# dannyfa/VAE-GAM

Hardware: AMD Instinct MI355X
Metric: fMRI volumes/sec/train-step (41x49x35) (higher is better)
Workload: dtype f32; 1 GPU; configs[2] full VAE-GAM: B=64/GPU C=8, 41x49x35, 2 subj x 98 vol synthetic checker, fwd+bwd+Adam, hipGraph replay; global_batch=64, covariates=8, parallelism=dp1

## Files before the change

include/vaegam.h:

```cpp
#ifndef VAEGAM_H
#define VAEGAM_H
#include <stdint.h>
#ifdef __cplusplus
extern "C" {
#endif

typedef struct vg_conv_desc {
    int32_t N;
    int32_t CI, CO;
    int32_t ID, IH, IW;
    int32_t OD, OH, OW;
    int32_t KD, KH, KW;
    int32_t stride;
    int32_t pad_d, pad_h, pad_w;
    int32_t relu_in;
    int32_t per_group;
} vg_conv_desc;

int         vg_version(void);
const char* vg_last_error(void);

int vg_corr3d(const vg_conv_desc* d, const float* x, const float* wpk, const float* bias,
              const float* in_scale, const float* in_shift, const float* mask_src, float* y, void* stream);

int vg_tconv3d_s2(const vg_conv_desc* d, const float* x, const float* wpk, const float* bias,
                  const float* in_scale, const float* in_shift, const float* mask_src, float* y, void* stream);
int64_t vg_tconv3d_s2_stats_chunks(const vg_conv_desc* d, int32_t stats_per_group);
int vg_tconv3d_s2_stats(const vg_conv_desc* d, const float* x, const float* wpk, const float* bias,
                        const float* in_scale, const float* in_shift, float* y, int32_t stats_per_group,
                        int32_t stats_relu, double* stats_part, void* stream);

typedef struct vg_mm_desc {
    int32_t N, CI, CO;
    int32_t ID, IH, IW, OD, OH, OW;
    int32_t nq, ks[4];
    int32_t PDT, PH, PW, PD;
    int32_t sdi, shi, swi, d0, LD, cc;
    int32_t sdo, sho, swo, od0[4], oh0[4], ow0[4];
    int32_t relu_in, per_group, tpc, slack;
    int32_t dbuf;
    int32_t PHB;
    int32_t hlo, hhi;
    int32_t waves;
} vg_mm_desc;
int64_t vg_conv_mm_stats_chunks(const vg_mm_desc* d, int32_t stats_per_group);
int vg_conv_mm(const vg_mm_desc* d, const float* x, const float* a_img, const int32_t* tau, const int32_t* dlt, const float* bias,
               const float* in_scale, const float* in_shift, const float* mask_src, float* y, int32_t stats_per_group,
               int32_t stats_relu, double* stats_part, void* stream);
int vg_gather_f32(const float* src, const int32_t* idx, float* dst, int64_t n, void* stream);

typedef struct vg_wgrad_desc {
    int32_t N, CB, CA;
    int32_t PD, PH, PW;
    int32_t AD, AH, AW;
    int32_t KD, KH, KW;
    int32_t stride;
    int32_t pad_d, pad_h, pad_w;
    int32_t pro_on_a;
    int32_t relu_in;
    int32_t per_group;
} vg_wgrad_desc;
int64_t vg_wgrad3d_ws_bytes(const vg_wgrad_desc* d);
int vg_wgrad3d(const vg_wgrad_desc* d, const float* a, const float* b, const float* in_scale,
               const float* in_shift, float* ws, float* dw, int32_t accumulate, void* stream);

int64_t vg_wgrad3d_grouped_ws_bytes(const vg_wgrad_desc* d);
int vg_wgrad3d_grouped(const vg_wgrad_desc* d, const float* a, const float* b, const float* in_scale,
                       const float* in_shift, float* ws, float* out, void* stream);

int64_t vg_bn_ws_bytes(int32_t N, int32_t C, int64_t P, int32_t per_group);
int vg_bn_stats(const float* x, int32_t N, int32_t C, int64_t P, int32_t per_group, int32_t relu,
                const float* gamma, const float* beta, float eps, void* ws, double* ext_sums,
                float* scale, float* shift, float* mean, float* rstd, void* stream);
int vg_bn_finalize(const double* sums, int32_t G, int32_t C, const float* gamma, const float* beta,
                   float eps, float* scale, float* shift, float* mean, float* rstd, void* stream);
int vg_bn_stats_from_parts(const double* part, int32_t G, int32_t C, int64_t chunks, double count,
                           const float* gamma, const float* beta, float eps, double* ext_sums, double* sums_ws,
                           float* scale, float* shift, float* mean, float* rstd, void* stream);

int vg_bn_bwd_reduce(const float* dxe, const float* p, int32_t N, int32_t C, int64_t P, int32_t per_group,
                     int32_t relu, const float* mean, const float* rstd, void* ws, double* sums, void* stream);
int vg_bn_bwd_apply(float* dxe_inout, const float* p, int32_t N, int32_t C, int64_t P, int32_t per_group,
                    int32_t relu, const float* gamma, const float* mean, const float* rstd,
                    const double* sums, double count, float* dgamma_part, float* dbeta_part,
                    void* ws, float* chsum, int32_t chsum_accumulate, void* stream);

int64_t vg_bn_tconv1_ws_bytes(int32_t N, int32_t C, int32_t ID, int32_t per_group);
int vg_bn_bwd_reduce_tconv1(const float* dy, const float* w, const float* p, int32_t N, int32_t C, int32_t ID, int32_t IH, int32_t IW,
                            int32_t per_group, int32_t relu, const float* mean, const float* rstd, void* ws, double* sums, void* stream);
int vg_bn_bwd_apply_tconv1(const float* dy, const float* w, const float* p, float* dp, int32_t N, int32_t C, int32_t ID, int32_t IH,
                           int32_t IW, int32_t per_group, int32_t relu, const float* gamma, const float* mean, const float* rstd,
                           const double* sums, double count, void* ws, float* chsum, int32_t chsum_accumulate, void* stream);

int vg_bn_tconv1_sums(const float* q, const float* w, const float* gamma, const float* beta, int32_t G, int32_t C, int32_t K,
                      double* sums, float* dw, int32_t accumulate, void* stream);

int vg_channel_sum(const float* x, int32_t N, int32_t C, int64_t P, void* ws, float* out, int32_t accumulate, void* stream);

int64_t vg_gam_ws_bytes(int32_t C, int32_t B, int64_t V);
int vg_gam_elbo_fwd(const float* logits, const float* gain, const float* x, const double* eps,
                    const float* glm, int32_t C, int32_t B, int64_t V, void* ws,
                    float* sum_log_prob, float* dist, float* maps_out, void* stream);
int vg_gam_elbo_bwd(const float* logits, const float* gain, const float* x, const double* eps,
                    const float* glm, const float* dist, const float* g_slp, const float* g_dist,
                    int32_t C, int32_t B, int64_t V, void* ws,
                    float* d_logits, float* d_gain, double* d_eps, float* d_total, int32_t total_accumulate, void* stream);

int vg_bn_param_grad(const double* sums, int32_t G, int32_t C, float* dgamma, float* dbeta, int32_t accumulate, void* stream);

int vg_data_bn_nshift(const float* mean, const float* rstd, int32_t n, float* nshift, void* stream);
int vg_data_bn_grads(const float* dw_hat, const float* db, const float* w, const float* gamma, const float* beta,
                     int32_t CO, int32_t CI, int32_t taps, float* dw, float* dbias, float* dgamma, float* dbeta,
                     int32_t accumulate, void* stream);

int vg_latent_fwd(const float* mu, const float* w, const float* a, const float* eps_w, const float* eps_d,
                  int32_t B, int32_t L, int32_t G, float* zcat, float* kl, float* d_out, float* flag_out, void* stream);
int vg_latent_bwd(const float* mu, const float* w, const float* d, const float* flag, const float* eps_w, const float* eps_d,
                  const float* g_zcat, const float* g_kl, int32_t B, int32_t L, int32_t G,
                  float* g_mu, float* g_w, float* g_a, void* stream);

int vg_loss_fwd(const float* kl, const float* slp, const float* dist, const float* gp_kl, int32_t B, int32_t CB,
                double c_kl, double c_slp, double c_gp, double c_dist, float* loss, void* stream);
int vg_loss_bwd(const float* g_loss, int32_t B, int32_t CB, double c_kl, double c_slp, double c_gp, double c_dist,
                float* g_kl, float* g_slp, float* g_dist, float* g_gp, void* stream);

int64_t vg_knn_ws_bytes(int32_t N, int32_t D, int32_t k);
int vg_knn(const float* x, int32_t N, int32_t D, int32_t k, void* ws, int32_t* idx, float* dist, void* stream);

int vg_umap_fuzzy(const float* dist, const int32_t* idx, int32_t N, int32_t k, double* ws, float* rho, float* sigma, float* w,
                  void* stream);

int vg_umap_layout_epoch(const int32_t* rowptr, const int32_t* col, const float* eps, const float* y_in, int32_t N, int32_t nnz,
                         int32_t epoch, int32_t n_epochs, double a, double b, int32_t negative_sample_rate, uint64_t seed,
                         float* y_out, void* stream);

enum { VG_FC_A_RELU = 1, VG_FC_A_MASK = 2, VG_FC_B_RELU = 4, VG_FC_B_ONES = 8, VG_FC_C_BIAS = 16, VG_FC_C_RELU = 32, VG_FC_C_MASK = 64,
       VG_FC_C_ACCUM = 128 };
typedef struct vg_fc_desc {
    int32_t M, N, K, batch;
    int64_t a_sm, a_sk, a_sb;
    int64_t b_sk, b_sn, b_sb;
    int64_t c_sm, c_sb;
    int64_t bias_sb, cx_sb;
    int32_t ksplit, flags;
} vg_fc_desc;
int64_t vg_fc_ws_bytes(const vg_fc_desc* d);
int vg_fc_gemm(const vg_fc_desc* d, const float* A, const float* amask, const float* B, const float* bias, const float* cmask,
               float* C, float* cx, float* ws, void* stream);
typedef struct vg_fc_job {
    vg_fc_desc d;
    const float *A, *amask, *B, *bias, *cmask;
    float *C, *cx, *ws;
} vg_fc_job;
int vg_fc_gemm_jobs(const vg_fc_job* jobs, int32_t njobs, void* stream);

int vg_pack_weights(const float* flat_params, float* packed, const int64_t* segs, int32_t nseg, int64_t total, void* stream);

int vg_cholesky_f64(const double* a, double* l, int32_t batch, int32_t n, void* stream);

typedef struct vg_gain_desc {
    int32_t C, B, n;
    int32_t hrf_taps;
    double jitter_b;
    double jitter_ku;
    double prior_var;
} vg_gain_desc;
int64_t vg_gp_gain_ws_bytes(int32_t C, int32_t B, int32_t n);
int vg_gp_gain_fwd(const vg_gain_desc* d, const int64_t* table, const float* params, const float* xu,
                   const float* covariates, int64_t ld_cov, const float* eps_beta, const double* hrf_taps, void* ws,
                   float* task_var, float* gp_kl, double* beta_mean, double* beta_cov, double* f_bar, double* Sigma, void* stream);
int vg_gp_gain_bwd(const vg_gain_desc* d, const int64_t* table, const float* params, const float* xu,
                   const float* covariates, int64_t ld_cov, const float* eps_beta, const double* hrf_taps, void* ws,
                   const float* g_task_var, const float* g_gp_kl, float* flat_grads, void* stream);
int vg_gp_gain_fwd_tiled(const vg_gain_desc* d, const int64_t* table, const float* params, const float* xu,
                         const float* covariates, int64_t ld_cov, const float* eps_beta, const double* hrf_taps, void* ws,
                         float* task_var, float* gp_kl, double* beta_mean, double* beta_cov, double* f_bar, double* Sigma, void* stream);
int vg_gp_gain_bwd_tiled(const vg_gain_desc* d, const int64_t* table, const float* params, const float* xu,
                         const float* covariates, int64_t ld_cov, const float* eps_beta, const double* hrf_taps, void* ws,
                         const float* g_task_var, const float* g_gp_kl, float* flat_grads, void* stream);

int vg_adam_advance(double* state, double lr, double b1, double b2, void* stream);
int vg_adam_step(void* p, const void* g, void* m, void* v, int64_t n, int32_t is_f64,
                 double b1, double b2, double eps, const double* step_scalars, void* stream);

#define VG_GUARD_STATE_LEN 8
int64_t vg_grad_guard_ws_bytes(int64_t n32, int64_t n64);
int vg_grad_guard(const float* g32, int64_t n32, const double* g64, int64_t n64, double max_norm, int32_t skip_nonfinite,
                  void* ws, double* state, void* stream);
int vg_adam_advance_guarded(double* state, double lr, double b1, double b2, const double* guard, void* stream);
int vg_adam_step_guarded(void* p, const void* g, void* m, void* v, int64_t n, int32_t is_f64,
                         double b1, double b2, double eps, const double* step_scalars, const double* guard, void* stream);

#ifdef __cplusplus
}
#endif
#endif
```

vae-gam_amd/_lib.py:

```python
import ctypes
import os

import torch

_HERE = os.path.dirname(os.path.abspath(__file__))
LIB_NAME = 'libvaegam_hip.so'

i32, i64, f32, f64, vp = ctypes.c_int32, ctypes.c_int64, ctypes.c_float, ctypes.c_double, ctypes.c_void_p


class ConvDesc(ctypes.Structure):
    _fields_ = [(n, i32) for n in ('N', 'CI', 'CO', 'ID', 'IH', 'IW', 'OD', 'OH', 'OW', 'KD', 'KH', 'KW',
                                   'stride', 'pad_d', 'pad_h', 'pad_w', 'relu_in', 'per_group')]


class WgradDesc(ctypes.Structure):
    _fields_ = [(n, i32) for n in ('N', 'CB', 'CA', 'PD', 'PH', 'PW', 'AD', 'AH', 'AW', 'KD', 'KH', 'KW',
                                   'stride', 'pad_d', 'pad_h', 'pad_w', 'pro_on_a', 'relu_in', 'per_group')]


class MmDesc(ctypes.Structure):
    _fields_ = [(n, i32) for n in ('N', 'CI', 'CO', 'ID', 'IH', 'IW', 'OD', 'OH', 'OW', 'nq')] + [('ks', i32 * 4)] + \
               [(n, i32) for n in ('PDT', 'PH', 'PW', 'PD', 'sdi', 'shi', 'swi', 'd0', 'LD', 'cc', 'sdo', 'sho', 'swo')] + \
               [('od0', i32 * 4), ('oh0', i32 * 4), ('ow0', i32 * 4)] + [(n, i32) for n in ('relu_in', 'per_group', 'tpc', 'slack', 'dbuf', 'PHB', 'hlo', 'hhi', 'waves')]


class GainDesc(ctypes.Structure):
    _fields_ = [('C', i32), ('B', i32), ('n', i32), ('hrf_taps', i32), ('jitter_b', f64), ('jitter_ku', f64), ('prior_var', f64)]


class FcDesc(ctypes.Structure):
    _fields_ = [('M', i32), ('N', i32), ('K', i32), ('batch', i32), ('a_sm', i64), ('a_sk', i64), ('a_sb', i64),
                ('b_sk', i64), ('b_sn', i64), ('b_sb', i64), ('c_sm', i64), ('c_sb', i64), ('bias_sb', i64), ('cx_sb', i64),
                ('ksplit', i32), ('flags', i32)]


class FcJob(ctypes.Structure):
    _fields_ = [('d', FcDesc), ('A', vp), ('amask', vp), ('B', vp), ('bias', vp), ('cmask', vp), ('C', vp), ('cx', vp), ('ws', vp)]


FC_A_RELU, FC_A_MASK, FC_B_RELU, FC_B_ONES, FC_C_BIAS, FC_C_RELU, FC_C_MASK, FC_C_ACCUM = 1, 2, 4, 8, 16, 32, 64, 128


_PROTOS = {
    'vg_version': (ctypes.c_int, []),
    'vg_last_error': (ctypes.c_char_p, []),
    'vg_corr3d': (ctypes.c_int, [ctypes.POINTER(ConvDesc), vp, vp, vp, vp, vp, vp, vp, vp]),
    'vg_tconv3d_s2': (ctypes.c_int, [ctypes.POINTER(ConvDesc), vp, vp, vp, vp, vp, vp, vp, vp]),
    'vg_tconv3d_s2_stats_chunks': (i64, [ctypes.POINTER(ConvDesc), i32]),
    'vg_tconv3d_s2_stats': (ctypes.c_int, [ctypes.POINTER(ConvDesc), vp, vp, vp, vp, vp, vp, i32, i32, vp, vp]),
    'vg_bn_stats_from_parts': (ctypes.c_int, [vp, i32, i32, i64, f64, vp, vp, f32, vp, vp, vp, vp, vp, vp, vp]),
    'vg_wgrad3d_ws_bytes': (i64, [ctypes.POINTER(WgradDesc)]),
    'vg_wgrad3d': (ctypes.c_int, [ctypes.POINTER(WgradDesc), vp, vp, vp, vp, vp, vp, i32, vp]),
    'vg_wgrad3d_grouped_ws_bytes': (i64, [ctypes.POINTER(WgradDesc)]),
    'vg_wgrad3d_grouped': (ctypes.c_int, [ctypes.POINTER(WgradDesc), vp, vp, vp, vp, vp, vp, vp]),
    'vg_bn_tconv1_sums': (ctypes.c_int, [vp, vp, vp, vp, i32, i32, i32, vp, vp, i32, vp]),
    'vg_bn_ws_bytes': (i64, [i32, i32, i64, i32]),
    'vg_bn_stats': (ctypes.c_int, [vp, i32, i32, i64, i32, i32, vp, vp, f32, vp, vp, vp, vp, vp, vp, vp]),
    'vg_bn_finalize': (ctypes.c_int, [vp, i32, i32, vp, vp, f32, vp, vp, vp, vp, vp]),
    'vg_bn_bwd_reduce': (ctypes.c_int, [vp, vp, i32, i32, i64, i32, i32, vp, vp, vp, vp, vp]),
    'vg_bn_bwd_apply': (ctypes.c_int, [vp, vp, i32, i32, i64, i32, i32, vp, vp, vp, vp, f64, vp, vp, vp, vp, i32, vp]),
    'vg_bn_tconv1_ws_bytes': (i64, [i32, i32, i32, i32]),
    'vg_bn_bwd_reduce_tconv1': (ctypes.c_int, [vp, vp, vp, i32, i32, i32, i32, i32, i32, i32, vp, vp, vp, vp, vp]),
    'vg_bn_bwd_apply_tconv1': (ctypes.c_int, [vp, vp, vp, vp, i32, i32, i32, i32, i32, i32, i32, vp, vp, vp, vp, f64, vp, vp, i32, vp]),
    'vg_bn_param_grad': (ctypes.c_int, [vp, i32, i32, vp, vp, i32, vp]),
    'vg_data_bn_nshift': (ctypes.c_int, [vp, vp, i32, vp, vp]),
    'vg_data_bn_grads': (ctypes.c_int, [vp, vp, vp, vp, vp, i32, i32, i32, vp, vp, vp, vp, i32, vp]),
    'vg_latent_fwd': (ctypes.c_int, [vp, vp, vp, vp, vp, i32, i32, i32, vp, vp, vp, vp, vp]),
    'vg_latent_bwd': (ctypes.c_int, [vp, vp, vp, vp, vp, vp, vp, vp, i32, i32, i32, vp, vp, vp, vp]),
    'vg_loss_fwd': (ctypes.c_int, [vp, vp, vp, vp, i32, i32, f64, f64, f64, f64, vp, vp]),
    'vg_loss_bwd': (ctypes.c_int, [vp, i32, i32, f64, f64, f64, f64, vp, vp, vp, vp, vp]),
    'vg_knn_ws_bytes': (i64, [i32, i32, i32]),
    'vg_knn': (ctypes.c_int, [vp, i32, i32, i32, vp, vp, vp, vp]),
    'vg_umap_fuzzy': (ctypes.c_int, [vp, vp, i32, i32, vp, vp, vp, vp, vp]),
    'vg_umap_layout_epoch': (ctypes.c_int, [vp, vp, vp, vp, i32, i32, i32, i32, f64, f64, i32, ctypes.c_uint64, vp, vp]),
    'vg_channel_sum': (ctypes.c_int, [vp, i32, i32, i64, vp, vp, i32, vp]),
    'vg_gam_ws_bytes': (i64, [i32, i32, i64]),
    'vg_gam_elbo_fwd': (ctypes.c_int, [vp, vp, vp, vp, vp, i32, i32, i64, vp, vp, vp, vp, vp]),
    'vg_gam_elbo_bwd': (ctypes.c_int, [vp, vp, vp, vp, vp, vp, vp, vp, i32, i32, i64, vp, vp, vp, vp, vp, i32, vp]),
    'vg_pack_weights': (ctypes.c_int, [vp, vp, vp, i32, i64, vp]),
    'vg_cholesky_f64': (ctypes.c_int, [vp, vp, i32, i32, vp]),
    'vg_conv_mm_stats_chunks': (i64, [ctypes.POINTER(MmDesc), i32]),
    'vg_conv_mm': (ctypes.c_int, [ctypes.POINTER(MmDesc), vp, vp, vp, vp, vp, vp, vp, vp, vp, i32, i32, vp, vp]),
    'vg_gather_f32': (ctypes.c_int, [vp, vp, vp, i64, vp]),
    'vg_fc_ws_bytes': (i64, [ctypes.POINTER(FcDesc)]),
    'vg_fc_gemm': (ctypes.c_int, [ctypes.POINTER(FcDesc), vp, vp, vp, vp, vp, vp, vp, vp, vp]),
    'vg_fc_gemm_jobs': (ctypes.c_int, [ctypes.POINTER(FcJob), i32, vp]),
    'vg_gp_gain_ws_bytes': (i64, [i32, i32, i32]),
    'vg_gp_gain_fwd': (ctypes.c_int, [ctypes.POINTER(GainDesc), vp, vp, vp, vp, i64, vp, vp, vp, vp, vp, vp, vp, vp, vp, vp]),
    'vg_gp_gain_bwd': (ctypes.c_int, [ctypes.POINTER(GainDesc), vp, vp, vp, vp, i64, vp, vp, vp, vp, vp, vp, vp]),
    'vg_gp_gain_fwd_tiled': (ctypes.c_int, [ctypes.POINTER(GainDesc), vp, vp, vp, vp, i64, vp, vp, vp, vp, vp, vp, vp, vp, vp, vp]),
    'vg_gp_gain_bwd_tiled': (ctypes.c_int, [ctypes.POINTER(GainDesc), vp, vp, vp, vp, i64, vp, vp, vp, vp, vp, vp, vp]),
    'vg_adam_advance': (ctypes.c_int, [vp, f64, f64, f64, vp]),
    'vg_adam_step': (ctypes.c_int, [vp, vp, vp, vp, i64, i32, f64, f64, f64, vp, vp]),
    'vg_grad_guard_ws_bytes': (i64, [i64, i64]),
    'vg_grad_guard': (ctypes.c_int, [vp, i64, vp, i64, f64, i32, vp, vp, vp]),
    'vg_adam_advance_guarded': (ctypes.c_int, [vp, f64, f64, f64, vp, vp]),
    'vg_adam_step_guarded': (ctypes.c_int, [vp, vp, vp, vp, i64, i32, f64, f64, f64, vp, vp, vp]),
}
GUARD_STATE_LEN = 8
EXPORTS = tuple(_PROTOS)


class VgError(RuntimeError):
    pass


class VgLibrary:
    host_pointers_ok = False

    def __init__(self, path):
        if not os.path.exists(path):
            raise VgError('HIP kernel library %s not found: run `python -c "import __graft_entry__ as g; g.build()"` '
                          '(hipcc --offload-arch=gfx950). There is no CPU fallback.' % path)
        self.path = path
        self.dll = ctypes.CDLL(path)
        for name, (res, args) in _PROTOS.items():
            fn = getattr(self.dll, name)
            fn.restype, fn.argtypes = res, args

    def call(self, name, *args):
        rc = getattr(self.dll, name)(*args)
        if rc != 0:
            raise VgError('%s failed (status %d): %s' % (name, rc, self.dll.vg_last_error().decode()))

    def size(self, name, *args):
        n = getattr(self.dll, name)(*args)
        if n < 0:
            raise VgError('%s: unsupported configuration: %s' % (name, self.dll.vg_last_error().decode()))
        return int(n)


_LIB = None


def library_path():
    return os.path.join(_HERE, LIB_NAME)


def get_lib() -> VgLibrary:
    global _LIB
    if _LIB is None:
        _LIB = VgLibrary(library_path())
    return _LIB
```

vae-gam_amd/csrc/vg_bn.hip:

```cpp
#include "vg_common.h"
#include "../../include/vaegam.h"

namespace {

constexpr int BN_THREADS = 256;
constexpr int BN_EPT = 16;

__device__ __forceinline__ double wave_sum(double v) {
#pragma unroll
    for (int off = 32; off > 0; off >>= 1) v += __shfl_down(v, off);
    return v;
}

__device__ __forceinline__ void block_sum2(double& a, double& b) {
    __shared__ double red[2][BN_THREADS / VG_WAVE];
    const int lane = threadIdx.x % VG_WAVE, wave = threadIdx.x / VG_WAVE;
    a = wave_sum(a); b = wave_sum(b);
    __syncthreads();
    if (lane == 0) { red[0][wave] = a; red[1][wave] = b; }
    __syncthreads();
    if (threadIdx.x == 0) {
        a = 0; b = 0;
        for (int w = 0; w < BN_THREADS / VG_WAVE; ++w) { a += red[0][w]; b += red[1][w]; }
    }
}

template <int MODE>
__global__ void __launch_bounds__(BN_THREADS)
bn_partial_k(const float* __restrict__ x, const float* __restrict__ p, const float* __restrict__ mean,
             const float* __restrict__ rstd, int C, long long P, int per_group, int relu, int cp, double* __restrict__ part) {
    const int chunk = blockIdx.x, c = blockIdx.y, g = blockIdx.z, chunks = gridDim.x;
    const int cpi = chunk % cp, si = chunk / cp, ns = chunks / cp;
    float mu = 0.f, rs = 1.f;
    if (MODE == 1) { mu = mean[g * C + c]; rs = rstd[g * C + c]; }
    float s0 = 0.f, s1 = 0.f;
    double d0 = 0.0, d1 = 0.0;
    int since = 0;
    for (int nn = si; nn < per_group; nn += ns) {
        const long long base = (((long long)g * per_group + nn) * C + c) * P;
        for (long long e = (long long)cpi * BN_THREADS + threadIdx.x; e < P; e += (long long)cp * BN_THREADS) {
            const long long off = base + e;
            if (MODE == 0) {
                float v = x[off];
                if (relu) v = fmaxf(v, 0.f);
                s0 += v; s1 = fmaf(v, v, s1);
            } else {
                float h = p[off];
                if (relu) h = fmaxf(h, 0.f);
                const float dv = x[off];
                s0 += dv; s1 = fmaf(dv, (h - mu) * rs, s1);
            }
            if (++since == 64) { d0 += s0; d1 += s1; s0 = 0.f; s1 = 0.f; since = 0; }
        }
    }
    d0 += s0; d1 += s1;
    block_sum2(d0, d1);
    if (threadIdx.x == 0) {
        part[((size_t)(g * C + c) * chunks + chunk) * 2 + 0] = d0;
        part[((size_t)(g * C + c) * chunks + chunk) * 2 + 1] = d1;
    }
}

__global__ void __launch_bounds__(BN_THREADS)
bn_fold_k(const double* __restrict__ part, int GC, int chunks, double count, int nout, double* __restrict__ sums) {
    const int i = blockIdx.x, lane = threadIdx.x;
    double a = 0, b = 0;
    for (int k = lane; k < chunks; k += BN_THREADS) { a += part[((size_t)i * chunks + k) * 2]; b += part[((size_t)i * chunks + k) * 2 + 1]; }
    block_sum2(a, b);
    if (lane == 0) {
        sums[(size_t)i * nout] = a; sums[(size_t)i * nout + 1] = b;
        if (nout == 3) sums[(size_t)i * nout + 2] = count;
    }
}

__global__ void bn_finalize_k(const double* __restrict__ sums, int G, int C, const float* __restrict__ gamma,
                              const float* __restrict__ beta, float eps, float* __restrict__ scale,
                              float* __restrict__ shift, float* __restrict__ mean, float* __restrict__ rstd) {
    const int i = blockIdx.x * blockDim.x + threadIdx.x;
    if (i >= G * C) return;
    const int c = i % C;
    const double cnt = sums[(size_t)i * 3 + 2];
    const double mu = sums[(size_t)i * 3] / cnt;
    double var = sums[(size_t)i * 3 + 1] / cnt - mu * mu;
    if (var < 0) var = 0;
    const float rs = (float)(1.0 / sqrt(var + (double)eps));
    const float gm = gamma ? gamma[c] : 1.f, bt = beta ? beta[c] : 0.f;
    const float sc = gm * rs;
    scale[i] = sc; shift[i] = bt - (float)mu * sc; mean[i] = (float)mu; rstd[i] = rs;
}

__global__ void __launch_bounds__(BN_THREADS)
bn_fold_finalize_k(const double* __restrict__ part, int C, int chunks, double count, const float* __restrict__ gamma,
                   const float* __restrict__ beta, float eps, float* __restrict__ scale, float* __restrict__ shift,
                   float* __restrict__ mean, float* __restrict__ rstd) {
    const int i = blockIdx.x, lane = threadIdx.x;
    double a = 0, b = 0;
    for (int k = lane; k < chunks; k += BN_THREADS) { a += part[((size_t)i * chunks + k) * 2]; b += part[((size_t)i * chunks + k) * 2 + 1]; }
    block_sum2(a, b);
    if (lane == 0) {
        const int c = i % C;
        const double mu = a / count;
        double var = b / count - mu * mu;
        if (var < 0) var = 0;
        const float rs = (float)(1.0 / sqrt(var + (double)eps));
        const float gm = gamma ? gamma[c] : 1.f, bt = beta ? beta[c] : 0.f;
        const float sc = gm * rs;
        scale[i] = sc; shift[i] = bt - (float)mu * sc; mean[i] = (float)mu; rstd[i] = rs;
    }
}

__global__ void __launch_bounds__(BN_THREADS)
bn_bwd_apply_k(float* __restrict__ dxe, const float* __restrict__ p, int C, long long P, int per_group, int relu,
               const float* __restrict__ gamma, const float* __restrict__ mean, const float* __restrict__ rstd,
               const double* __restrict__ sums, double count, int cp, float* __restrict__ dgamma_part, float* __restrict__ dbeta_part,
               double* __restrict__ csum_part) {
    const int chunk = blockIdx.x, c = blockIdx.y, g = blockIdx.z, chunks = gridDim.x;
    const int cpi = chunk % cp, si = chunk / cp, ns = chunks / cp;
    const int gc = g * C + c;
    const float mu = mean[gc], rs = rstd[gc];
    const float m1 = (float)(sums[(size_t)gc * 2] / count), m2 = (float)(sums[(size_t)gc * 2 + 1] / count);
    const float k = (gamma ? gamma[c] : 1.f) * rs;
    if (chunk == 0 && threadIdx.x == 0) {
        dbeta_part[gc] = (float)sums[(size_t)gc * 2];
        dgamma_part[gc] = (float)sums[(size_t)gc * 2 + 1];
    }
    float vs = 0.f;
    for (int nn = si; nn < per_group; nn += ns) {
        const long long base = (((long long)g * per_group + nn) * C + c) * P;
        for (long long e = (long long)cpi * BN_THREADS + threadIdx.x; e < P; e += (long long)cp * BN_THREADS) {
            const long long off = base + e;
            const float pv = p[off];
            const float h = relu ? fmaxf(pv, 0.f) : pv;
            const float hh = (h - mu) * rs;
            float v = k * (dxe[off] - m1 - hh * m2);
            if (relu && !(pv > 0.f)) v = 0.f;
            dxe[off] = v;
            vs += v;
        }
    }
    if (csum_part) {
        double a = (double)vs, b = 0.0;
        block_sum2(a, b);
        if (threadIdx.x == 0) csum_part[(size_t)gc * chunks + chunk] = a;
    }
}

__global__ void __launch_bounds__(BN_THREADS)
csum_fold_k(const double* __restrict__ part, int G, int C, int chunks, int accumulate, float* __restrict__ out) {
    const int c = blockIdx.x, lane = threadIdx.x;
    double a = 0, unused = 0;
    for (int g = 0; g < G; ++g)
        for (int k = lane; k < chunks; k += BN_THREADS) a += part[((size_t)g * C + c) * chunks + k];
    block_sum2(a, unused);
    if (lane == 0) out[c] = (accumulate ? out[c] : 0.f) + (float)a;
}

struct BnPlan { int cp, ns; int chunks() const { return cp * ns; } };
BnPlan plan_for(long long P, int per_group, int C, int G) {
    BnPlan b;
    long long c = (P + (long long)BN_THREADS * BN_EPT - 1) / ((long long)BN_THREADS * BN_EPT);
    if (c < 1) c = 1;
    if (c > 64) c = 64;
    b.cp = (int)c;
    long long want = 2048 / ((long long)b.cp * C * G);
    if (want < 1) want = 1;
    if (want > per_group) want = per_group;
    if (want > 64) want = 64;
    b.ns = (int)want;
    return b;
}

}

extern "C" int64_t vg_bn_ws_bytes(int32_t N, int32_t C, int64_t P, int32_t per_group) {
    if (N <= 0 || C <= 0 || P <= 0 || per_group <= 0 || N % per_group) return -1;
    const int G = N / per_group;
    const int chunks = plan_for(P, per_group, C, G).chunks();
    return (int64_t)G * C * chunks * 2 * sizeof(double) + (int64_t)G * C * 3 * sizeof(double);
}

static int bn_args_ok(const char* who, const void* x, int N, int C, long long P, int per_group) {
    if (!x || N <= 0 || C <= 0 || P <= 0 || per_group <= 0 || N % per_group) {
        vg_set_error("%s: bad arguments N=%d C=%d P=%lld per_group=%d", who, N, C, P, per_group); return VG_ERR_ARG;
    }
    if (C > 65535 || N / per_group > 65535) { vg_set_error("%s: grid limit", who); return VG_ERR_ARG; }
    return VG_OK;
}

extern "C" int vg_bn_finalize(const double* sums, int32_t G, int32_t C, const float* gamma, const float* beta,
                              float eps, float* scale, float* shift, float* mean, float* rstd, void* stream) {
    if (!sums || !scale || !shift || !mean || !rstd || G <= 0 || C <= 0) { vg_set_error("vg_bn_finalize: bad arguments"); return VG_ERR_ARG; }
    vg_launch(bn_finalize_k, dim3(vg_cdiv(G * C, 64)), dim3(64), 0, (hipStream_t)stream, sums, G, C, gamma, beta, eps, scale, shift, mean, rstd);
    return vg_check_launch("bn_finalize");
}

extern "C" int vg_bn_stats(const float* x, int32_t N, int32_t C, int64_t P, int32_t per_group, int32_t relu,
                           const float* gamma, const float* beta, float eps, void* ws, double* ext_sums,
                           float* scale, float* shift, float* mean, float* rstd, void* stream) {
    int rc = bn_args_ok("vg_bn_stats", x, N, C, P, per_group);
    if (rc) return rc;
    if (!ws) { vg_set_error("vg_bn_stats: null workspace"); return VG_ERR_ARG; }
    hipStream_t s = (hipStream_t)stream;
    const int G = N / per_group;
    const long long total = (long long)per_group * P;
    const BnPlan pl = plan_for(P, per_group, C, G);
    const int chunks = pl.chunks();
    double* part = (double*)ws;
    double* sums = ext_sums ? ext_sums : part + (size_t)G * C * chunks * 2;
    vg_launch(bn_partial_k<0>, dim3(chunks, C, G), dim3(BN_THREADS), 0, s, x, (const float*)nullptr, (const float*)nullptr,
              (const float*)nullptr, (int)C, (long long)P, (int)per_group, (int)relu, pl.cp, part);
    if ((rc = vg_check_launch("bn_partial"))) return rc;
    if (!ext_sums) {
        if (!scale || !shift || !mean || !rstd) { vg_set_error("vg_bn_stats: null output"); return VG_ERR_ARG; }
        vg_launch(bn_fold_finalize_k, dim3(G * C), dim3(BN_THREADS), 0, s, (const double*)part, (int)C, chunks, (double)total, gamma, beta, eps,
                  scale, shift, mean, rstd);
        return vg_check_launch("bn_fold_finalize");
    }
    vg_launch(bn_fold_k, dim3(G * C), dim3(BN_THREADS), 0, s, (const double*)part, G * C, chunks, (double)total, 3, sums);
    return vg_check_launch("bn_fold");
}

extern "C" int vg_bn_bwd_reduce(const float* dxe, const float* p, int32_t N, int32_t C, int64_t P, int32_t per_group,
                                int32_t relu, const float* mean, const float* rstd, void* ws, double* sums, void* stream) {
    int rc = bn_args_ok("vg_bn_bwd_reduce", dxe, N, C, P, per_group);
    if (rc) return rc;
    if (!p || !mean || !rstd || !ws || !sums) { vg_set_error("vg_bn_bwd_reduce: null argument"); return VG_ERR_ARG; }
    hipStream_t s = (hipStream_t)stream;
    const int G = N / per_group;
    const long long total = (long long)per_group * P;
    const BnPlan pl = plan_for(P, per_group, C, G);
    const int chunks = pl.chunks();
    double* part = (double*)ws;
    vg_launch(bn_partial_k<1>, dim3(chunks, C, G), dim3(BN_THREADS), 0, s, dxe, p, mean, rstd, (int)C, (long long)P,
              (int)per_group, (int)relu, pl.cp, part);
    if ((rc = vg_check_launch("bn_bwd_partial"))) return rc;
    vg_launch(bn_fold_k, dim3(G * C), dim3(BN_THREADS), 0, s, (const double*)part, G * C, chunks, (double)total, 2, sums);
    return vg_check_launch("bn_bwd_fold");
}

extern "C" int vg_bn_bwd_apply(float* dxe, const float* p, int32_t N, int32_t C, int64_t P, int32_t per_group,
                               int32_t relu, const float* gamma, const float* mean, const float* rstd,
                               const double* sums, double count, float* dgamma_part, float* dbeta_part,
                               void* ws, float* chsum, int32_t chsum_accumulate, void* stream) {
    int rc = bn_args_ok("vg_bn_bwd_apply", dxe, N, C, P, per_group);
    if (rc) return rc;
    if (!p || !mean || !rstd || !sums || !dgamma_part || !dbeta_part || !(count > 0)) { vg_set_error("vg_bn_bwd_apply: bad argument"); return VG_ERR_ARG; }
    if (chsum && !ws) { vg_set_error("vg_bn_bwd_apply: chsum needs the vg_bn_ws_bytes workspace"); return VG_ERR_ARG; }
    const int G = N / per_group;
    const BnPlan pl = plan_for(P, per_group, C, G);
    double* csum_part = chsum ? (double*)ws : nullptr;
    vg_launch(bn_bwd_apply_k, dim3(pl.chunks(), C, G), dim3(BN_THREADS), 0, (hipStream_t)stream, dxe, p, (int)C, (long long)P,
              (int)per_group, (int)relu, gamma, mean, rstd, sums, count, pl.cp, dgamma_part, dbeta_part, csum_part);
    if ((rc = vg_check_launch("bn_bwd_apply"))) return rc;
    if (chsum) {
        vg_launch(csum_fold_k, dim3(C), dim3(BN_THREADS), 0, (hipStream_t)stream, (const double*)csum_part, G, (int)C, pl.chunks(),
                  (int)chsum_accumulate, chsum);
        return vg_check_launch("bn_bwd csum_fold");
    }
    return VG_OK;
}

namespace {
constexpr int FT_TD = 3;
constexpr int FT_MAXC = 16;

struct FtParams {
    int N, C, ID, IH, IW;
    int per_group, relu, tilesD;
    float inv_iw, inv_plane;
};

#ifdef VG_EMU
static inline float to_vgpr(float v) { return v; }
#else
__device__ __forceinline__ float to_vgpr(float v) { float r; asm volatile("v_mov_b32 %0, %1" : "=v"(r) : "s"(v)); return r; }
#endif

template <int MODE, int CT>
__global__ void __launch_bounds__(BN_THREADS)
bn_tconv1_k(const float* __restrict__ dy, const float* __restrict__ w, const float* __restrict__ p, float* __restrict__ dp,
            const float* __restrict__ gamma, const float* __restrict__ mean, const float* __restrict__ rstd,
            const double* __restrict__ sums, double count, FtParams a, double* __restrict__ part, double* __restrict__ csum_part) {
    VG_DYN_SMEM(float, tile);
    const int tid = threadIdx.x, lane = tid % VG_WAVE, wave = vg_wave_id();
    const int n = blockIdx.y, td = blockIdx.x;
    const int C = CT ? CT : a.C;
    const int g = n / a.per_group;
    const int OH = a.IH + 2, OW = a.IW + 2, oplane = OH * OW, iplane = a.IH * a.IW;
    const int d0 = td * FT_TD, nd = min(FT_TD, a.ID - d0);
    {
        const float* src = dy + ((size_t)n * (a.ID + 2) + d0) * oplane;
        const int nfl = (nd + 2) * oplane;
        vg_dma_block(src, tile, nfl, wave, BN_THREADS / VG_WAVE, lane);
        vg_dma_wait();
    }
    __syncthreads();
    float mu[CT ? CT : FT_MAXC], rs[CT ? CT : FT_MAXC], k1[CT ? CT : FT_MAXC], m1[CT ? CT : FT_MAXC], m2[CT ? CT : FT_MAXC];
    float acc0[CT ? CT : FT_MAXC], acc1[CT ? CT : FT_MAXC];
#pragma unroll
    for (int c = 0; c < (CT ? CT : FT_MAXC); ++c) {
        if (c < C) {
            const int gc = g * C + c;
            mu[c] = to_vgpr(mean[gc]); rs[c] = to_vgpr(rstd[gc]);
            if (MODE == 1) {
                m1[c] = to_vgpr((float)(sums[(size_t)gc * 2] / count)); m2[c] = to_vgpr((float)(sums[(size_t)gc * 2 + 1] / count));
                k1[c] = to_vgpr((gamma ? gamma[c] : 1.f) * rstd[gc]);
            }
        }
        acc0[c] = 0.f; acc1[c] = 0.f;
    }
    const int npos = nd * iplane;
    const float lo = a.relu ? 0.f : -__builtin_inff();
    const size_t vol = (size_t)a.ID * iplane;
    const float* pb = p + (size_t)n * C * vol + (size_t)d0 * iplane;
    float* dpb = MODE == 1 ? dp + (size_t)n * C * vol + (size_t)d0 * iplane : nullptr;
    constexpr int PP = 2;
    for (int e0 = tid; e0 < npos; e0 += PP * BN_THREADS) {
        int ee[PP]; bool ok[PP]; int toff[PP];
#pragma unroll
        for (int u = 0; u < PP; ++u) {
            const int e = e0 + u * BN_THREADS;
            ok[u] = e < npos;
            ee[u] = ok[u] ? e : e0;
            int dl = (int)((float)ee[u] * a.inv_plane);
            int r = ee[u] - dl * iplane;
            dl += (r >= iplane ? 1 : 0) - (r < 0 ? 1 : 0);
            r = ee[u] - dl * iplane;
            int h = (int)((float)r * a.inv_iw);
            int x = r - h * a.IW;
            h += (x >= a.IW ? 1 : 0) - (x < 0 ? 1 : 0);
            x = r - h * a.IW;
            toff[u] = dl * oplane + h * OW + x;
        }
        float pv[PP][CT ? CT : FT_MAXC];
#pragma unroll
        for (int u = 0; u < PP; ++u)
#pragma unroll
            for (int c = 0; c < (CT ? CT : FT_MAXC); ++c) if (c < C) pv[u][c] = pb[(size_t)c * vol + ee[u]];
        float win[PP][27];
#pragma unroll
        for (int u = 0; u < PP; ++u) {
            const float* t0 = tile + toff[u];
#pragma unroll
            for (int kd = 0; kd < 3; ++kd)
#pragma unroll
                for (int kh = 0; kh < 3; ++kh) {
                    const float* row = t0 + kd * oplane + kh * OW;
#pragma unroll
                    for (int kw = 0; kw < 3; ++kw) win[u][(kd * 3 + kh) * 3 + kw] = row[kw];
                }
        }
        float wcur[27], wnxt[27];
        {
            vg_cptr w0 = VG_CPTR(w);
#pragma unroll
            for (int k = 0; k < 27; ++k) wcur[k] = w0[k];
        }
#pragma unroll
        for (int c = 0; c < (CT ? CT : FT_MAXC); ++c) {
            if (c >= C) continue;
#ifndef VG_EMU
            __builtin_amdgcn_sched_barrier(0);
#endif
            if (c + 1 < C) {
                int coff = (c + 1) * 27;
#ifndef VG_EMU
                asm volatile("" : "+s"(coff));
#endif
                vg_cptr wn = VG_CPTR(w) + coff;
#pragma unroll
                for (int k = 0; k < 27; ++k) wnxt[k] = wn[k];
            }
            float dxe[PP];
#pragma unroll
            for (int u = 0; u < PP; ++u) dxe[u] = 0.f;
#pragma unroll
            for (int k = 0; k < 27; ++k) {
#pragma unroll
                for (int u = 0; u < PP; ++u) dxe[u] = fmaf(win[u][k], wcur[k], dxe[u]);
            }
#pragma unroll
            for (int u = 0; u < PP; ++u) {
                const float hv = vg_max(pv[u][c], lo);
                const float hh = (hv - mu[c]) * rs[c];
                if (MODE == 0) {
                    const float dm = ok[u] ? dxe[u] : 0.f;
                    acc0[c] += dm; acc1[c] = fmaf(dm, hh, acc1[c]);
                } else {
                    float v = k1[c] * (dxe[u] - m1[c] - hh * m2[c]);
                    v = (pv[u][c] > lo) ? v : 0.f;
                    if (ok[u]) { dpb[(size_t)c * vol + ee[u]] = v; acc0[c] += v; }
                }
            }
#pragma unroll
            for (int k = 0; k < 27; ++k) wcur[k] = wnxt[k];
        }
    }
    __shared__ double red[2][FT_MAXC][BN_THREADS / VG_WAVE];
    const int chunks = a.per_group * a.tilesD;
    const int chunk = (n % a.per_group) * a.tilesD + td;
#pragma unroll
    for (int c = 0; c < (CT ? CT : FT_MAXC); ++c) {
        if (c >= C) continue;
        const double s0 = wave_sum((double)acc0[c]);
        const double s1 = MODE == 0 ? wave_sum((double)acc1[c]) : 0.0;
        if (lane == 0) { red[0][c][wave] = s0; red[1][c][wave] = s1; }
    }
    __syncthreads();
    if (tid < C) {
        double s0 = 0, s1 = 0;
        for (int wv = 0; wv < BN_THREADS / VG_WAVE; ++wv) { s0 += red[0][tid][wv]; s1 += red[1][tid][wv]; }
        const size_t gc = (size_t)g * C + tid;
        if (MODE == 0) { part[(gc * chunks + chunk) * 2] = s0; part[(gc * chunks + chunk) * 2 + 1] = s1; }
        else if (csum_part) csum_part[gc * chunks + chunk] = s0;
    }
}

static int ft_setup(const char* who, const float* dy, const float* w, const float* p, int N, int C, int ID, int IH, int IW, int per_group,
                    FtParams* a, size_t* shmem) {
    if (!dy || !w || !p || N <= 0 || C <= 0 || C > FT_MAXC || ID <= 0 || IH <= 0 || IW <= 0 || per_group <= 0 || N % per_group || N > 65535) {
        vg_set_error("%s: bad arguments N=%d C=%d p=%dx%dx%d per_group=%d", who, N, C, ID, IH, IW, per_group); return VG_ERR_ARG;
    }
    a->N = N; a->C = C; a->ID = ID; a->IH = IH; a->IW = IW; a->per_group = per_group; a->relu = 0;
    a->tilesD = vg_cdiv(ID, FT_TD);
    a->inv_iw = 1.0f / (float)IW; a->inv_plane = 1.0f / (float)(IH * IW);
    *shmem = (size_t)(FT_TD + 2) * (IH + 2) * (IW + 2) * sizeof(float) + 256;
    if (*shmem > 150 * 1024) { vg_set_error("%s: a %dx%d dy plane tile does not fit LDS", who, IH + 2, IW + 2); return VG_ERR_UNSUPPORTED; }
    if ((long long)FT_TD * IH * IW >= (1 << 22)) { vg_set_error("%s: tile too large for the position decode", who); return VG_ERR_UNSUPPORTED; }
    return VG_OK;
}

}

extern "C" int64_t vg_bn_tconv1_ws_bytes(int32_t N, int32_t C, int32_t ID, int32_t per_group) {
    if (N <= 0 || C <= 0 || ID <= 0 || per_group <= 0 || N % per_group) return -1;
    const int64_t chunks = (int64_t)per_group * vg_cdiv(ID, FT_TD);
    return (int64_t)(N / per_group) * C * chunks * 2 * (int64_t)sizeof(double);
}

extern "C" int vg_bn_bwd_reduce_tconv1(const float* dy, const float* w, const float* p, int32_t N, int32_t C, int32_t ID, int32_t IH,
                                       int32_t IW, int32_t per_group, int32_t relu, const float* mean, const float* rstd, void* ws,
                                       double* sums, void* stream) {
    FtParams a; size_t shmem;
    int rc = ft_setup("vg_bn_bwd_reduce_tconv1", dy, w, p, N, C, ID, IH, IW, per_group, &a, &shmem);
    if (rc) return rc;
    if (!mean || !rstd || !ws || !sums) { vg_set_error("vg_bn_bwd_reduce_tconv1: null argument"); return VG_ERR_ARG; }
    a.relu = relu;
    hipStream_t s = (hipStream_t)stream;
    const int G = N / per_group, chunks = per_group * a.tilesD;
    double* part = (double*)ws;
    if (C == 8)
        vg_launch(bn_tconv1_k<0, 8>, dim3(a.tilesD, N), dim3(BN_THREADS), shmem, s, dy, w, p, (float*)nullptr, (const float*)nullptr, mean, rstd,
                  (const double*)nullptr, 1.0, a, part, (double*)nullptr);
    else
        vg_launch(bn_tconv1_k<0, 0>, dim3(a.tilesD, N), dim3(BN_THREADS), shmem, s, dy, w, p, (float*)nullptr, (const float*)nullptr, mean, rstd,
                  (const double*)nullptr, 1.0, a, part, (double*)nullptr);
    if ((rc = vg_check_launch("bn_bwd_reduce_tconv1"))) return rc;
    vg_launch(bn_fold_k, dim3(G * C), dim3(BN_THREADS), 0, s, (const double*)part, G * C, chunks, (double)per_group * ID * IH * IW, 2, sums);
    return vg_check_launch("bn_bwd_reduce_tconv1 fold");
}

__global__ void __launch_bounds__(256)
bn_tconv1_sums_k(const float* __restrict__ q, const float* __restrict__ w, const float* __restrict__ gamma,
                 const float* __restrict__ beta, int G, int C, int K, double* __restrict__ sums, float* __restrict__ dw, int accumulate) {
    for (int i = threadIdx.x; i < G * C; i += blockDim.x) {
        const int g = i / C, c = i % C;
        const float* Q = q + ((size_t)g * (C + 1) + c) * K;
        const float* S = q + ((size_t)g * (C + 1) + C) * K;
        double s0 = 0, s1 = 0;
        for (int k = 0; k < K; ++k) { const double wv = w[c * K + k]; s0 += wv * S[k]; s1 += wv * Q[k]; }
        sums[(size_t)i * 2] = s0; sums[(size_t)i * 2 + 1] = s1;
    }
    for (int j = threadIdx.x; j < C * K; j += blockDim.x) {
        const int c = j / K, k = j % K;
        double a = 0, b = 0;
        for (int g = 0; g < G; ++g) { a += q[((size_t)g * (C + 1) + c) * K + k]; b += q[((size_t)g * (C + 1) + C) * K + k]; }
        const float v = (float)((double)gamma[c] * a + (double)beta[c] * b);
        dw[j] = accumulate ? dw[j] + v : v;
    }
}

extern "C" int vg_bn_tconv1_sums(const float* q, const float* w, const float* gamma, const float* beta, int32_t G, int32_t C, int32_t K,
                                 double* sums, float* dw, int32_t accumulate, void* stream) {
    if (!q || !w || !gamma || !beta || !sums || !dw || G <= 0 || C <= 0 || K <= 0) { vg_set_error("vg_bn_tconv1_sums: bad argument"); return VG_ERR_ARG; }
    vg_launch(bn_tconv1_sums_k, dim3(1), dim3(256), 0, (hipStream_t)stream, q, w, gamma, beta, (int)G, (int)C, (int)K, sums, dw, (int)accumulate);
    return vg_check_launch("bn_tconv1_sums");
}

extern "C" int vg_bn_bwd_apply_tconv1(const float* dy, const float* w, const float* p, float* dp, int32_t N, int32_t C, int32_t ID,
                                      int32_t IH, int32_t IW, int32_t per_group, int32_t relu, const float* gamma, const float* mean,
                                      const float* rstd, const double* sums, double count, void* ws, float* chsum,
                                      int32_t chsum_accumulate, void* stream) {
    FtParams a; size_t shmem;
    int rc = ft_setup("vg_bn_bwd_apply_tconv1", dy, w, p, N, C, ID, IH, IW, per_group, &a, &shmem);
    if (rc) return rc;
    if (!dp || !mean || !rstd || !sums || !(count > 0) || (chsum && !ws)) { vg_set_error("vg_bn_bwd_apply_tconv1: bad argument"); return VG_ERR_ARG; }
    a.relu = relu;
    hipStream_t s = (hipStream_t)stream;
    const int G = N / per_group, chunks = per_group * a.tilesD;
    double* csum_part = chsum ? (double*)ws : nullptr;
    if (C == 8)
        vg_launch(bn_tconv1_k<1, 8>, dim3(a.tilesD, N), dim3(BN_THREADS), shmem, s, dy, w, p, dp, gamma, mean, rstd, sums, count, a,
                  (double*)nullptr, csum_part);
    else
        vg_launch(bn_tconv1_k<1, 0>, dim3(a.tilesD, N), dim3(BN_THREADS), shmem, s, dy, w, p, dp, gamma, mean, rstd, sums, count, a,
                  (double*)nullptr, csum_part);
    if ((rc = vg_check_launch("bn_bwd_apply_tconv1"))) return rc;
    if (chsum) {
        vg_launch(csum_fold_k, dim3(C), dim3(BN_THREADS), 0, s, (const double*)csum_part, G, (int)C, chunks, (int)chsum_accumulate, chsum);
        return vg_check_launch("bn_bwd_apply_tconv1 csum_fold");
    }
    return VG_OK;
}

namespace {
__global__ void __launch_bounds__(BN_THREADS)
chsum_fold_k(const double* __restrict__ part, int C, int chunks, int accumulate, float* __restrict__ out) {
    const int c = blockIdx.x, lane = threadIdx.x;
    double a = 0, unused = 0;
    for (int k = lane; k < chunks; k += BN_THREADS) a += part[((size_t)c * chunks + k) * 2];
    block_sum2(a, unused);
    if (lane == 0) out[c] = (accumulate ? out[c] : 0.f) + (float)a;
}
}

extern "C" int vg_channel_sum(const float* x, int32_t N, int32_t C, int64_t P, void* ws, float* out, int32_t accumulate, void* stream) {
    int rc = bn_args_ok("vg_channel_sum", x, N, C, P, N);
    if (rc) return rc;
    if (!ws || !out) { vg_set_error("vg_channel_sum: null argument"); return VG_ERR_ARG; }
    hipStream_t s = (hipStream_t)stream;
    const BnPlan pl = plan_for(P, N, C, 1);
    const int chunks = pl.chunks();
    double* part = (double*)ws;
    vg_launch(bn_partial_k<0>, dim3(chunks, C, 1), dim3(BN_THREADS), 0, s, x, (const float*)nullptr, (const float*)nullptr,
              (const float*)nullptr, (int)C, (long long)P, (int)N, 0, pl.cp, part);
    if ((rc = vg_check_launch("channel_sum partial"))) return rc;
    vg_launch(chsum_fold_k, dim3(C), dim3(BN_THREADS), 0, s, (const double*)part, (int)C, chunks, (int)accumulate, out);
    return vg_check_launch("channel_sum fold");
}

extern "C" int vg_bn_stats_from_parts(const double* part, int32_t G, int32_t C, int64_t chunks, double count,
                                      const float* gamma, const float* beta, float eps, double* ext_sums, double* sums_ws,
                                      float* scale, float* shift, float* mean, float* rstd, void* stream) {
    if (!part || G <= 0 || C <= 0 || chunks <= 0 || !(count > 0)) { vg_set_error("vg_bn_stats_from_parts: bad argument"); return VG_ERR_ARG; }
    hipStream_t s = (hipStream_t)stream;
    if (!ext_sums) {
        if (!scale || !shift || !mean || !rstd) { vg_set_error("vg_bn_stats_from_parts: null output"); return VG_ERR_ARG; }
        vg_launch(bn_fold_finalize_k, dim3(G * C), dim3(BN_THREADS), 0, s, part, (int)C, (int)chunks, count, gamma, beta, eps, scale, shift, mean, rstd);
        return vg_check_launch("bn_fold_finalize(parts)");
    }
    vg_launch(bn_fold_k, dim3(G * C), dim3(BN_THREADS), 0, s, part, G * C, (int)chunks, count, 3, ext_sums);
    return vg_check_launch("bn_fold(parts)");
}

namespace {
__global__ void __launch_bounds__(64)
bn_param_grad_k(const double* __restrict__ sums, int G, int C, int accumulate, float* __restrict__ dgamma, float* __restrict__ dbeta) {
    const int c = blockIdx.x * blockDim.x + threadIdx.x;
    if (c >= C) return;
    double a = 0, b = 0;
    for (int g = 0; g < G; ++g) { b += sums[((size_t)g * C + c) * 2]; a += sums[((size_t)g * C + c) * 2 + 1]; }
    dgamma[c] = (accumulate ? dgamma[c] : 0.f) + (float)a;
    dbeta[c] = (accumulate ? dbeta[c] : 0.f) + (float)b;
}
__global__ void __launch_bounds__(256)
data_bn_grads_k(const float* __restrict__ dw_hat, const float* __restrict__ db, const float* __restrict__ w,
                const float* __restrict__ gamma, const float* __restrict__ beta, int CO, int CI, int T, int acc,
                float* __restrict__ dw, float* __restrict__ dbias, float* __restrict__ dgamma, float* __restrict__ dbeta) {
    __shared__ float red[2][256];
    const int tid = threadIdx.x, n = CO * CI * T;
    for (int i = tid; i < n; i += 256) {
        const int co = i / (CI * T), ci = (i / T) % CI;
        const float v = gamma[ci] * dw_hat[i] + beta[ci] * db[co];
        dw[i] = acc ? dw[i] + v : v;
    }
    for (int co = tid; co < CO; co += 256) dbias[co] = acc ? dbias[co] + db[co] : db[co];
    for (int ci = 0; ci < CI; ++ci) {
        float sg = 0.f, sb = 0.f;
        for (int i = tid; i < CO * T; i += 256) {
            const int co = i / T, t = i - co * T;
            const float wv = w[((size_t)co * CI + ci) * T + t];
            sg += wv * dw_hat[((size_t)co * CI + ci) * T + t];
            sb += wv * db[co];
        }
        red[0][tid] = sg; red[1][tid] = sb;
        __syncthreads();
        for (int o = 128; o > 0; o >>= 1) {
            if (tid < o) { red[0][tid] += red[0][tid + o]; red[1][tid] += red[1][tid + o]; }
            __syncthreads();
        }
        if (tid == 0) {
            dgamma[ci] = acc ? dgamma[ci] + red[0][0] : red[0][0];
            dbeta[ci] = acc ? dbeta[ci] + red[1][0] : red[1][0];
        }
        __syncthreads();
    }
}

__global__ void data_bn_nshift_k(const float* __restrict__ mean, const float* __restrict__ rstd, int n, float* __restrict__ out) {
    const int i = blockIdx.x * blockDim.x + threadIdx.x;
    if (i < n) out[i] = -(mean[i] * rstd[i]);
}

}

extern "C" int vg_data_bn_nshift(const float* mean, const float* rstd, int32_t n, float* nshift, void* stream) {
    if (!mean || !rstd || !nshift || n <= 0) { vg_set_error("vg_data_bn_nshift: bad argument"); return VG_ERR_ARG; }
    vg_launch(data_bn_nshift_k, dim3(vg_cdiv(n, 64)), dim3(64), 0, (hipStream_t)stream, mean, rstd, (int)n, nshift);
    return vg_check_launch("data_bn_nshift");
}

extern "C" int vg_data_bn_grads(const float* dw_hat, const float* db, const float* w, const float* gamma, const float* beta,
                                int32_t CO, int32_t CI, int32_t taps, float* dw, float* dbias, float* dgamma, float* dbeta,
                                int32_t accumulate, void* stream) {
    if (!dw_hat || !db || !w || !gamma || !beta || !dw || !dbias || !dgamma || !dbeta || CO <= 0 || CI <= 0 || taps <= 0) {
        vg_set_error("vg_data_bn_grads: bad argument"); return VG_ERR_ARG;
    }
    vg_launch(data_bn_grads_k, dim3(1), dim3(256), 0, (hipStream_t)stream, dw_hat, db, w, gamma, beta, (int)CO, (int)CI, (int)taps,
              (int)accumulate, dw, dbias, dgamma, dbeta);
    return vg_check_launch("data_bn_grads");
}

extern "C" int vg_bn_param_grad(const double* sums, int32_t G, int32_t C, float* dgamma, float* dbeta, int32_t accumulate,
                                void* stream) {
    if (!sums || !dgamma || !dbeta || G <= 0 || C <= 0) { vg_set_error("vg_bn_param_grad: bad argument"); return VG_ERR_ARG; }
    vg_launch(bn_param_grad_k, dim3(vg_cdiv(C, 64)), dim3(64), 0, (hipStream_t)stream, sums, (int)G, (int)C, (int)accumulate, dgamma,
              dbeta);
    return vg_check_launch("bn_param_grad");
}
```

vae-gam_amd/csrc/vg_conv_mm.hip:

```cpp
#include "vg_common.h"
#include <stdlib.h>
#include <stdint.h>
#include "../../include/vaegam.h"

#ifdef VG_STAMP
__device__ unsigned long long vg_stamp_out[1024 * 16 * 8];
#define VG_STAMP_T(t) do { __builtin_amdgcn_sched_barrier(0); asm volatile("s_memtime %0\n\ts_waitcnt lgkmcnt(0)" : "=s"(t) :: "memory"); __builtin_amdgcn_sched_barrier(0); } while (0)
#define VG_STAMP_ADD(i) do { unsigned long long t_; VG_STAMP_T(t_); st_sum[i] += t_ - st_last; st_last = t_; } while (0)
#else
#define VG_STAMP_ADD(i) do {} while (0)
#endif

namespace {

constexpr int MM_MAXQ = 4;
constexpr int MM_ZPAD = 64;

struct MmParams {
    vg_mm_desc d;
    int bps, nsplit;
    int ksbase[MM_MAXQ], a_off[MM_MAXQ];
    int kstot, aimg_floats;
    int a_res;
    int CHP, buf_floats;
    int nhb, PHB, h0, LH, LPH;
    int tau_off, in_off;
    int has_pro;
};

struct alignas(16) mm_f4 { float v[4]; };

template <int V> struct mm_int { static constexpr int value = V; };
template <int MAXN, typename F>
__device__ __forceinline__ void mm_dispatch(int n, F&& f) {
    if constexpr (MAXN >= 1) {
        if (n == MAXN) { f(mm_int<MAXN>{}); return; }
        mm_dispatch<MAXN - 1>(n, f);
    }
}
template <int N, int I = 0, typename F>
__device__ __forceinline__ void mm_static_for(F&& f) {
    if constexpr (I < N) { f(mm_int<I>{}); mm_static_for<N, I + 1>(f); }
}

template <int MM_W, int NQ, int TPC, int K0, int K1, int K2, int K3, bool DB, int OCC, bool MASKED>
__global__ void __launch_bounds__(MM_W * VG_WAVE, OCC)
conv_mm_k(const float* __restrict__ x, const float* __restrict__ a_img, const int* __restrict__ tau, const int* __restrict__ dlt,
          const float* __restrict__ bias, const float* __restrict__ in_scale, const float* __restrict__ in_shift,
          const float* __restrict__ mask_src, float* __restrict__ y, double* __restrict__ stats_part, int stats_pg, int stats_relu,
          MmParams p) {
    VG_DYN_SMEM(float, lds);
    constexpr int MM_T = MM_W * VG_WAVE;
    const vg_mm_desc& d = p.d;
    float* Al = lds;
    int* Tl = reinterpret_cast<int*>(lds + p.tau_off);
    float* In = lds + p.in_off;
    const int tid = threadIdx.x, lane = tid % VG_WAVE, wave = vg_wave_id();
    const int kk = lane >> 4, jl = lane & 15;
    const int b = blockIdx.x % p.bps, split = blockIdx.x / p.bps;
    const int IHW = d.IH * d.IW, OHW = d.OH * d.OW;
    const int CI = d.CI, CO = d.CO;
    constexpr bool STATIC_K = K0 > 0;
    constexpr int KSUM = K0 + K1 + K2 + K3;

    for (int i = tid; i < p.aimg_floats; i += MM_T) Al[i] = a_img[i];
    if (!STATIC_K) for (int i = tid; i < p.kstot * 64; i += MM_T) {
        const int* e = dlt + ((i >> 6) * 4 + ((i & 63) >> 4)) * 3;
        Tl[i] = e[0] * p.LPH + e[1] * d.IW + e[2];
    }
    for (int i = tid; i < (DB ? 2 : 1) * d.cc * MM_ZPAD; i += MM_T) In[(i / MM_ZPAD) * p.CHP + (i % MM_ZPAD)] = 0.f;

    const int bd = b / p.nhb, bh = b - bd * p.nhb;
    const int pd0 = bd * d.PD, ph0 = bh * p.PHB;
    const int npd = min(d.PD, d.PDT - pd0), nph = min(p.PHB, d.PH - ph0);
    const int npos = npd * nph * d.PW;
    const int ntiles = (npos + 15) / 16;
    const int dlo = pd0 * d.sdi + d.d0;
    const int pl_lo = max(dlo, 0), pl_hi = min(dlo + d.LD, d.ID);
    const int npl = max(pl_hi - pl_lo, 0);
    const int rlo = ph0 * d.shi + p.h0;
    const int r_lo = max(rlo, 0), r_hi = min(rlo + p.LH, d.IH);
    const int LPH = p.LPH;
    const bool flat = (r_lo == 0 && r_hi == d.IH && LPH == IHW);
    const int span_fl = flat ? npl * IHW : max(r_hi - r_lo, 0) * d.IW;
    const int nspan_c = flat ? 1 : npl;
    const int dst0 = (pl_lo - dlo) * LPH;
    const size_t vol = (size_t)IHW * d.ID, ovol = (size_t)OHW * d.OD;
    const int rho_l = (CO == 8) ? (kk >> 1) : 0;
    const int co_l = (CO == 8) ? ((kk & 1) * 4) : kk * 4;
    int ob[TPC];
    unsigned vbits = 0;
    int pt[TPC][STATIC_K ? KSUM : 1];
    int posBase[TPC]; unsigned vm[NQ][TPC];
#pragma unroll
    for (int i = 0; i < TPC; ++i) {
        const int pf = (i * MM_W + wave) * 16 + jl;
        const bool pv = pf < npos;
        const int pfc = pv ? pf : 0;
        const int pdl = pfc / (nph * d.PW), r2 = pfc - pdl * (nph * d.PW);
        const int phl = r2 / d.PW, pw = r2 - phl * d.PW;
        const int ph = ph0 + phl;
        const int obd = (pd0 + pdl) * d.sdo, obh = ph * d.sho, obw = pw * d.swo + rho_l;
        ob[i] = obd * OHW + obh * d.OW + obw + co_l * (int)ovol;
#pragma unroll
        for (int q = 0; q < NQ; ++q) {
            const int od = obd + d.od0[q], oh = obh + d.oh0[q], ow = obw + d.ow0[q];
            const bool ok = pv && od >= 0 && od < d.OD && oh >= 0 && oh < d.OH && ow >= 0 && ow < d.OW;
            vbits |= (ok ? 1u : 0u) << (q * TPC + i);
        }
        const int pb = (pdl * d.sdi - d.d0) * LPH + (ph * d.shi - r_lo) * d.IW + pw * d.swi;
        posBase[i] = pb;
        if constexpr (STATIC_K) {
#pragma unroll
            for (int sg = 0; sg < KSUM; ++sg) {
                const int* e = dlt + (sg * 4 + kk) * 3;
                const int id = (pd0 + pdl) * d.sdi + e[0], ih = ph * d.shi + e[1], iw = pw * d.swi + e[2];
                const bool ok = pv && id >= 0 && id < d.ID && ih >= 0 && ih < d.IH && iw >= 0 && iw < d.IW;
                pt[i][sg] = ok ? MM_ZPAD + pb + e[0] * LPH + e[1] * d.IW + e[2] : 0;
            }
        } else {
#pragma unroll
            for (int q = 0; q < NQ; ++q) {
                unsigned m = 0;
                for (int s = 0; s < d.ks[q]; ++s) {
                    const int* e = dlt + ((p.ksbase[q] + s) * 4 + kk) * 3;
                    const int id = (pd0 + pdl) * d.sdi + e[0], ih = ph * d.shi + e[1], iw = pw * d.swi + e[2];
                    const bool ok = pv && id >= 0 && id < d.ID && ih >= 0 && ih < d.IH && iw >= 0 && iw < d.IW;
                    m |= (ok ? 1u : 0u) << s;
                }
                vm[q][i] = m;
            }
        }
    }
    const float lo = d.relu_in ? 0.f : -__builtin_inff();
    const int nchunks = (CI + d.cc - 1) / d.cc;
    const int nsamp = (d.N - split + p.nsplit - 1) / p.nsplit;
    const int units = nsamp * nchunks;

    vg_f32x4 acc[TPC];
    float st_s[4] = {0.f, 0.f, 0.f, 0.f}, st_q[4] = {0.f, 0.f, 0.f, 0.f};
    float mreg[MASKED ? TPC : 1][4];
    float bias_l[4];
#pragma unroll
    for (int r = 0; r < 4; ++r) bias_l[r] = bias ? bias[co_l + r] : 0.f;
    int nact = 0;
#pragma unroll
    for (int i = 0; i < TPC; ++i) nact += (i * MM_W + wave < ntiles) ? 1 : 0;

    int nst[NQ];
#pragma unroll
    for (int q = 0; q < NQ; ++q) {
        int c4 = 0;
#pragma unroll
        for (int i = 0; i < TPC; ++i) c4 += (vg_any(((vbits >> (q * TPC + i)) & 1u) != 0) && i < nact) ? 4 : 0;
        nst[q] = c4;
    }

    auto zero_acc = [&]() __attribute__((always_inline)) {
#pragma unroll
        for (int i = 0; i < TPC; ++i) { acc[i].v[0] = 0.f; acc[i].v[1] = 0.f; acc[i].v[2] = 0.f; acc[i].v[3] = 0.f; }
    };
    auto load_mask = [&](int n) __attribute__((always_inline)) {
        const char* mn = reinterpret_cast<const char*>(mask_src + (size_t)n * CO * ovol);
#pragma unroll
        for (int i = 0; i < TPC; ++i) {
            const bool okt = i < nact && ((vbits >> i) & 1u);
            const unsigned off = okt ? 4u * (unsigned)(ob[i] + d.od0[0] * OHW + d.oh0[0] * d.OW + d.ow0[0]) : 0u;
#pragma unroll
            for (int r = 0; r < 4; ++r)
                mreg[i][r] = okt ? *reinterpret_cast<const float*>(mn + (size_t)r * ovol * 4 + off) : 0.f;
        }
    };
    auto store_class = [&](int n, int q) __attribute__((always_inline)) {
        char* yn = reinterpret_cast<char*>(y + (size_t)n * CO * ovol);
        const char* mn = reinterpret_cast<const char*>(mask_src + (size_t)n * CO * ovol);
        const int cq = d.od0[q] * OHW + d.oh0[q] * d.OW + d.ow0[q];
#pragma unroll
        for (int i = 0; i < TPC; ++i) {
            if (i >= nact || !((vbits >> (q * TPC + i)) & 1u)) continue;
            const unsigned off = 4u * (unsigned)(ob[i] + cq);
#pragma unroll
            for (int r = 0; r < 4; ++r) {
                float v = acc[i].v[r] + bias_l[r];
                if constexpr (MASKED) {
                    if constexpr (NQ == 1) v = (mreg[i][r] > 0.f) ? v : 0.f;
                    else v = (*reinterpret_cast<const float*>(mn + (size_t)r * ovol * 4 + off) > 0.f) ? v : 0.f;
                }
#if defined(VG_ABLATE_STORE) && VG_ABLATE_STORE == 1
                if (v == 1.2345e-30f) *reinterpret_cast<float*>(yn + (size_t)r * ovol * 4 + off) = v;
#elif defined(VG_ABLATE_STORE) && VG_ABLATE_STORE == 2
                *reinterpret_cast<float*>(yn + (size_t)r * ovol * 4 + (((off >> 8) << 8) + 4u * lane)) = v;
#elif defined(VG_ABLATE_STORE) && VG_ABLATE_STORE == 4
                if (r == 0 || v == 1.2345e-30f) *reinterpret_cast<float*>(yn + (size_t)r * ovol * 4 + off) = v;
#elif defined(VG_ABLATE_STORE) && VG_ABLATE_STORE == 5
                *reinterpret_cast<float*>(yn + off) = v;
#elif defined(VG_ABLATE_STORE) && VG_ABLATE_STORE == 3
                __builtin_nontemporal_store(v, reinterpret_cast<float*>(yn + (size_t)r * ovol * 4 + off));
#else
                *reinterpret_cast<float*>(yn + (size_t)r * ovol * 4 + off) = v;
#endif
                if (stats_part) {
                    const float h = stats_relu ? vg_max(v, 0.f) : v;
                    st_s[r] += h; st_q[r] = fmaf(h, h, st_q[r]);
                }
            }
        }
    };
    auto flush_stats = [&](int n) __attribute__((always_inline)) {
        const int g = n / stats_pg;
        const size_t chunks = (size_t)stats_pg * p.bps * MM_W;
        const size_t chunkid = ((size_t)(n % stats_pg) * p.bps + b) * MM_W + wave;
#pragma unroll
        for (int r = 0; r < 4; ++r) {
            float sa = st_s[r], sb = st_q[r];
#pragma unroll
            for (int off = 8; off > 0; off >>= 1) { sa += __shfl_xor(sa, off); sb += __shfl_xor(sb, off); }
            if (CO == 8) { sa += __shfl_xor(sa, 32); sb += __shfl_xor(sb, 32); }
            if (jl == 0 && (CO == 16 || kk < 2)) {
                double* dst = stats_part + (((size_t)g * CO + co_l + r) * chunks + chunkid) * 2;
                dst[0] = (double)sa; dst[1] = (double)sb;
            }
            st_s[r] = 0.f; st_q[r] = 0.f;
        }
    };

    const int nsp = d.cc * nspan_c;
    const int parts = (nsp >= MM_W) ? 1 : (MM_W + nsp - 1) / nsp;
    const int head = dst0 & 3;
    const int n4 = (head + span_fl + 3) >> 2;
    const int n4p = (n4 + parts - 1) / parts;
    auto stage = [&](int u) __attribute__((always_inline)) {
        const int n = split + (u / nchunks) * p.nsplit, c0 = (u % nchunks) * d.cc;
        const int cc = min(d.cc, CI - c0);
        float* buf = In + (DB ? (u & 1) : 0) * p.buf_floats;
        const float* src0 = x + ((size_t)n * CI + c0) * vol + (size_t)pl_lo * IHW + (size_t)r_lo * d.IW;
        for (int it = wave; it < cc * nspan_c * parts; it += MM_W) {
            const int sp = it / parts, part = it - sp * parts;
            const int c = sp / nspan_c, pl = sp - c * nspan_c;
            const int g0 = part * n4p, g1 = min(g0 + n4p, n4);
            const int f0 = max(g0 * 4 - head, 0), f1 = min(g1 * 4 - head, span_fl);
            if (f1 > f0) vg_dma_block(src0 + (size_t)c * vol + (size_t)pl * IHW + f0, buf + c * p.CHP + MM_ZPAD + dst0 + pl * LPH + f0, f1 - f0, 0, 1, lane);
        }
    };
    auto prologue = [&](int u) __attribute__((always_inline)) {
        const int n = split + (u / nchunks) * p.nsplit, c0 = (u % nchunks) * d.cc;
        const int cc = min(d.cc, CI - c0);
        float* buf = In + (DB ? (u & 1) : 0) * p.buf_floats;
        const int g_aff = (in_scale != nullptr) ? n / d.per_group : 0;
        for (int it = wave; it < cc * nspan_c * parts; it += MM_W) {
            const int sp = it / parts, part = it - sp * parts;
            const int c = sp / nspan_c, pl = sp - c * nspan_c;
            float sc = 1.f, sh = 0.f;
            if (in_scale != nullptr) { sc = in_scale[g_aff * CI + c0 + c]; sh = in_shift[g_aff * CI + c0 + c]; }
            float* sp0 = buf + c * p.CHP + MM_ZPAD + dst0 + pl * LPH - head;
            const int g0 = part * n4p, g1 = min((part + 1) * n4p, n4);
#ifdef VG_EMU
            for (int g = g0 + lane; g < g1; g += VG_WAVE) {
                float* t = sp0 + g * 4;
#pragma unroll
                for (int e = 0; e < 4; ++e) t[e] = fmaf(vg_max(t[e], lo), sc, sh);
            }
#else
            for (int g = g0 + lane; g < g1; g += VG_WAVE) {
                const unsigned a = (unsigned)(uintptr_t)(sp0 + g * 4);
                vg_hw_f32x4 t;
                asm volatile("ds_read_b128 %0, %1\n\ts_waitcnt lgkmcnt(0)" : "=v"(t) : "v"(a) : "memory");
#pragma unroll
                for (int e = 0; e < 4; ++e) t[e] = fmaf(vg_max(t[e], lo), sc, sh);
                asm volatile("ds_write_b128 %0, %1" :: "v"(a), "v"(t) : "memory");
            }
#endif
        }
#ifndef VG_EMU
        asm volatile("s_waitcnt lgkmcnt(0)" ::: "memory");
#endif
    };
    __syncthreads();
#ifdef VG_STAMP
    unsigned long long st_sum[8] = {0, 0, 0, 0, 0, 0, 0, 0}, st_last;
    VG_STAMP_T(st_last);
#endif
    if (units > 0) stage(0);
    int g_run = -1, n_run = 0;
    int pend = 0;
    for (int u = 0; u < units; ++u) {
        const int n = split + (u / nchunks) * p.nsplit, chunk = u % nchunks, c0 = chunk * d.cc;
        const int cc = min(d.cc, CI - c0);
        float* cur = In + (DB ? (u & 1) : 0) * p.buf_floats;
        VG_STAMP_ADD(7);
        if (DB) vg_dma_wait_wave();
        else vg_wait_vm(pend);
        VG_STAMP_ADD(0);
        if (p.has_pro) prologue(u);
        VG_STAMP_ADD(1);
        __syncthreads();
        VG_STAMP_ADD(2);
        if (DB && u + 1 < units) stage(u + 1);
        if constexpr (NQ == 1 && MASKED) { if (chunk == nchunks - 1) load_mask(n); }
        VG_STAMP_ADD(3);
        auto class_work = [&](auto qc, auto ntc) __attribute__((always_inline)) {
            constexpr int q = decltype(qc)::value;
            constexpr int NT = decltype(ntc)::value;
            for (int c = 0; c < cc; ++c) {
                const float* curc = cur + c * p.CHP;
                if constexpr (STATIC_K) {
                    constexpr int KSQ = q == 0 ? K0 : q == 1 ? K1 : q == 2 ? K2 : K3;
                    constexpr int SG0 = q == 0 ? 0 : q == 1 ? K0 : q == 2 ? K0 + K1 : K0 + K1 + K2;
                    const float* Aq = Al + p.a_off[q] + (c0 + c) * KSQ * 64 + lane;
#ifdef VG_EMU
#pragma unroll
                    for (int s = 0; s < KSQ; ++s) {
                        const float aw = Aq[s * 64];
#pragma unroll
                        for (int i = 0; i < NT; ++i) vg_mfma16(aw, curc[pt[i][SG0 + s]], acc[i]);
                    }
#else
                    const unsigned cb = (unsigned)(uintptr_t)curc, ab = (unsigned)(uintptr_t)Aq;
                    float a2[2], b2[2][NT];
                    asm volatile("ds_read_b32 %0, %1" : "=v"(a2[0]) : "v"(ab));
#pragma unroll
                    for (int i = 0; i < NT; ++i) asm volatile("ds_read_b32 %0, %1" : "=v"(b2[0][i]) : "v"(cb + 4u * (unsigned)pt[i][SG0]));
#pragma unroll
                    for (int s = 0; s < KSQ; ++s) {
                        if (s + 1 < KSQ) {
                            asm volatile("ds_read_b32 %0, %1 offset:%2" : "=v"(a2[(s + 1) & 1]) : "v"(ab), "n"((s + 1) * 256));
#pragma unroll
                            for (int i = 0; i < NT; ++i)
                                asm volatile("ds_read_b32 %0, %1" : "=v"(b2[(s + 1) & 1][i]) : "v"(cb + 4u * (unsigned)pt[i][SG0 + s + 1]));
                            asm volatile("s_waitcnt lgkmcnt(%0)" :: "n"(NT + 1) : "memory");
                        } else {
                            asm volatile("s_waitcnt lgkmcnt(0)" ::: "memory");
                        }
                        __builtin_amdgcn_sched_barrier(0);
#pragma unroll
                        for (int i = 0; i < NT; ++i) vg_mfma16(a2[s & 1], b2[s & 1][i], acc[i]);
                        __builtin_amdgcn_sched_barrier(0);
                    }
#endif
                } else {
                    const int ksq = d.ks[q];
                    const float* Aq = Al + p.a_off[q] + (c0 + c) * ksq * 64 + lane;
                    const int* Tq = Tl + p.ksbase[q] * 64 + lane;
                    for (int s = 0; s < ksq; ++s) {
                        const float aw = Aq[s * 64];
                        const int off = Tq[s * 64] + MM_ZPAD;
                        const unsigned bit = 1u << s;
                        float bv[NT];
#pragma unroll
                        for (int i = 0; i < NT; ++i) bv[i] = curc[(vm[q][i] & bit) ? posBase[i] + off : 0];
#pragma unroll
                        for (int i = 0; i < NT; ++i) vg_mfma16(aw, bv[i], acc[i]);
                    }
                }
            }
        };
        const int g_now = stats_part ? n / stats_pg : 0;
        if (stats_part && chunk == 0 && g_run >= 0 && g_now != g_run) flush_stats(n_run);
        if constexpr (NQ == 1) {
            if (chunk == 0) zero_acc();
            if (nact > 0) mm_dispatch<TPC>(nact, [&](auto ntc) __attribute__((always_inline)) { class_work(mm_int<0>{}, ntc); });
            VG_STAMP_ADD(4);
            pend = 0;
            if constexpr (!DB) {
                if (u + 1 < units) { __syncthreads(); VG_STAMP_ADD(2); stage(u + 1); VG_STAMP_ADD(3); }
                if (chunk == nchunks - 1) pend = nst[0];
            }
            if (chunk == nchunks - 1) store_class(n, 0);
            VG_STAMP_ADD(5);
        } else {
            mm_static_for<NQ>([&](auto qc) __attribute__((always_inline)) {
                constexpr int q = decltype(qc)::value;
                zero_acc();
                VG_STAMP_ADD(5);
                if (nact > 0) mm_dispatch<TPC>(nact, [&](auto ntc) __attribute__((always_inline)) { class_work(qc, ntc); });
                VG_STAMP_ADD(4);
                if constexpr (!DB && q == NQ - 1) {
                    if (u + 1 < units) { __syncthreads(); VG_STAMP_ADD(2); stage(u + 1); VG_STAMP_ADD(3); }
                    pend = nst[q];
                }
                store_class(n, q);
            });
            VG_STAMP_ADD(5);
        }
        g_run = g_now; n_run = n;
    }
    if (stats_part && g_run >= 0) flush_stats(n_run);
    VG_STAMP_ADD(6);
#ifdef VG_STAMP
    if (lane == 0 && blockIdx.x < 1024)
        for (int i = 0; i < 8; ++i) vg_stamp_out[(blockIdx.x * 16 + wave) * 8 + i] = st_sum[i];
#endif
}

}

#ifdef VG_STAMP
extern "C" int vg_stamp_read(unsigned long long* dst, int n) {
    return (int)hipMemcpyFromSymbol(dst, HIP_SYMBOL(vg_stamp_out), sizeof(unsigned long long) * n, 0, hipMemcpyDeviceToHost);
}
#endif

static int mm_plan_params(const vg_mm_desc* d, MmParams* p, size_t* shmem, const char* who) {
    if (!d || d->N <= 0 || d->CI <= 0 || (d->CO != 8 && d->CO != 16) || d->nq < 1 || d->nq > MM_MAXQ || d->PD <= 0 || d->PDT <= 0 ||
        d->PH <= 0 || d->PW <= 0 || d->slack < 0 || d->PH > 1023 || d->PW > 1023 || d->PD > 1023 || d->cc <= 0 || d->LD <= 0 || d->tpc <= 0) {
        vg_set_error("%s: bad descriptor", who); return VG_ERR_ARG;
    }
    p->d = *d;
    int ns = 256 / p->bps; if (ns < 1) ns = 1; if (ns > d->N) ns = d->N;
    p->nsplit = ns;
    int row = 0, af = 0;
    for (int q = 0; q < d->nq; ++q) {
        if (d->ks[q] <= 0 || d->ks[q] > 32) { vg_set_error("%s: k-steps per channel must be 1..32 (class %d: %d)", who, q, d->ks[q]); return VG_ERR_ARG; }
        p->ksbase[q] = row; p->a_off[q] = af;
        row += d->ks[q]; af += d->CI * d->ks[q] * 64;
    }
    p->kstot = row; p->aimg_floats = af;
    if (d->nq > 1 && d->cc < d->CI) { vg_set_error("%s: multi-class plans need all input channels in one chunk", who); return VG_ERR_ARG; }
    const int IHW = d->IH * d->IW;
    const int W = d->waves;
    if (W != 4 && W != 8) { vg_set_error("%s: waves per workgroup must be 4 or 8 (got %d)", who, W); return VG_ERR_ARG; }
    if (d->hhi < d->hlo) { vg_set_error("%s: bad row-offset range [%d, %d]", who, d->hlo, d->hhi); return VG_ERR_ARG; }
    p->PHB = (d->PHB > 0 && d->PHB < d->PH) ? d->PHB : d->PH;
    p->nhb = vg_cdiv(d->PH, p->PHB);
    p->h0 = d->hlo;
    p->LH = (p->PHB - 1) * d->shi + (d->hhi - d->hlo) + 1;
    const int rows_max = p->LH < d->IH ? p->LH : d->IH;
    const bool whole = p->PHB == d->PH && d->hlo <= 0 && (d->PH - 1) * d->shi + d->hhi + 1 >= d->IH;
    p->LPH = whole ? IHW : ((rows_max * d->IW + 3) / 4) * 4 + 4;
    p->CHP = MM_ZPAD + ((d->LD * p->LPH + 63) / 64) * 64;
    p->buf_floats = d->cc * p->CHP;
    p->a_res = 1;
    p->tau_off = ((p->aimg_floats + 63) / 64) * 64;
    p->in_off = p->tau_off + p->kstot * 64;
    p->bps = vg_cdiv(d->PDT, d->PD) * p->nhb;
    const size_t total = (size_t)p->in_off + (d->dbuf ? 2 : 1) * (size_t)p->buf_floats + 64;
    *shmem = total * sizeof(float);
    if (*shmem > 160 * 1024) { vg_set_error("%s: plan needs %zu bytes of LDS", who, *shmem); return VG_ERR_UNSUPPORTED; }
    if (d->PD * p->PHB * d->PW > d->tpc * W * 16) { vg_set_error("%s: %d positions per block exceed tpc=%d x %d waves", who, d->PD * p->PHB * d->PW, d->tpc, W); return VG_ERR_ARG; }
    return VG_OK;
}

extern "C" int64_t vg_conv_mm_stats_chunks(const vg_mm_desc* d, int32_t stats_per_group) {
    if (!d || stats_per_group <= 0 || d->PD <= 0 || d->PDT <= 0 || d->PH <= 0 || (d->waves != 4 && d->waves != 8)) return -1;
    const int PHB = (d->PHB > 0 && d->PHB < d->PH) ? d->PHB : d->PH;
    return (int64_t)stats_per_group * vg_cdiv(d->PDT, d->PD) * vg_cdiv(d->PH, PHB) * d->waves;
}

extern "C" int vg_conv_mm(const vg_mm_desc* d, const float* x, const float* a_img, const int32_t* tau, const int32_t* dlt,
                          const float* bias, const float* in_scale, const float* in_shift, const float* mask_src, float* y,
                          int32_t stats_per_group, int32_t stats_relu, double* stats_part, void* stream) {
    MmParams p; size_t shmem;
    int rc = mm_plan_params(d, &p, &shmem, "vg_conv_mm");
    if (rc) return rc;
    if (!x || !a_img || !tau || !dlt || !y) { vg_set_error("vg_conv_mm: null argument"); return VG_ERR_ARG; }
    if ((in_scale == nullptr) != (in_shift == nullptr) || (in_scale && d->per_group <= 0)) { vg_set_error("vg_conv_mm: in_scale/in_shift/per_group inconsistent"); return VG_ERR_ARG; }
    if (stats_part && (stats_per_group <= 0 || d->N % stats_per_group)) { vg_set_error("vg_conv_mm: bad statistics arguments"); return VG_ERR_ARG; }
    p.has_pro = (d->relu_in || in_scale) ? 1 : 0;
    hipStream_t s = (hipStream_t)stream;
    const int threads = d->waves * VG_WAVE;
    auto launch = [&](auto kernel) {
        const int bpc = vg_blocks_per_cu((const void*)kernel, threads, shmem);
        int ns = (256 * bpc) / p.bps; if (ns < 1) ns = 1; if (ns > d->N) ns = d->N;
        p.nsplit = ns;
        vg_launch(kernel, dim3(p.bps * p.nsplit), dim3(threads), shmem, s, x, a_img, (const int*)tau, (const int*)dlt, bias, in_scale, in_shift,
                  mask_src, y, stats_part, (int)(stats_part ? stats_per_group : 1), (int)stats_relu, p);
    };
    const bool db = d->dbuf != 0, mk = mask_src != nullptr, w4 = d->waves == 4;
#define MM_LAUNCH_W(W, NQ, TPC, K0, K1, K2, K3) { \
        constexpr int OCC_ = (TPC * (K0 + K1 + K2 + K3) + 10 * TPC <= 96 && K0 > 0) ? 4 : 2; \
        if (db) { if (mk) launch(conv_mm_k<W, NQ, TPC, K0, K1, K2, K3, true, OCC_, true>); else launch(conv_mm_k<W, NQ, TPC, K0, K1, K2, K3, true, OCC_, false>); } \
        else    { if (mk) launch(conv_mm_k<W, NQ, TPC, K0, K1, K2, K3, false, OCC_, true>); else launch(conv_mm_k<W, NQ, TPC, K0, K1, K2, K3, false, OCC_, false>); } }
#define MM_LAUNCH(NQ, TPC, K0, K1, K2, K3) { if (w4) MM_LAUNCH_W(4, NQ, TPC, K0, K1, K2, K3) else MM_LAUNCH_W(8, NQ, TPC, K0, K1, K2, K3) }
#define MM_TPC(NQ, K0, K1, K2, K3) \
    { if (d->tpc <= 3) MM_LAUNCH(NQ, 3, K0, K1, K2, K3) else if (d->tpc <= 4) MM_LAUNCH(NQ, 4, K0, K1, K2, K3) else if (d->tpc <= 5) MM_LAUNCH(NQ, 5, K0, K1, K2, K3) \
      else if (d->tpc <= 6) MM_LAUNCH(NQ, 6, K0, K1, K2, K3) else MM_LAUNCH(NQ, 8, K0, K1, K2, K3) }
    const int* k = d->ks;
    if (d->nq == 1 && d->tpc <= 8) {
        if (k[0] == 7) MM_TPC(1, 7, 0, 0, 0)
        else if (k[0] == 9) MM_TPC(1, 9, 0, 0, 0)
        else if (k[0] == 12) MM_TPC(1, 12, 0, 0, 0)
        else if (k[0] == 19 && d->tpc <= 3) MM_LAUNCH(1, 3, 19, 0, 0, 0)
        else MM_TPC(1, 0, 0, 0, 0)
    } else if (d->nq == 4 && d->tpc <= 4) {
        if (k[0] == 3 && k[1] == 2 && k[2] == 2 && k[3] == 1) MM_LAUNCH(4, 4, 3, 2, 2, 1)
        else if (k[0] == 2 && k[1] == 1 && k[2] == 1 && k[3] == 1) MM_LAUNCH(4, 4, 2, 1, 1, 1)
        else if (k[0] == 2 && k[1] == 2 && k[2] == 2 && k[3] == 2) MM_LAUNCH(4, 4, 2, 2, 2, 2)
        else MM_LAUNCH(4, 4, 0, 0, 0, 0)
    } else { vg_set_error("vg_conv_mm: no kernel instance for %d classes x %d tiles per wave", d->nq, d->tpc); return VG_ERR_UNSUPPORTED; }
#undef MM_TPC
#undef MM_LAUNCH
#undef MM_LAUNCH_W
    return vg_check_launch("conv_mm");
}

namespace {
__global__ void __launch_bounds__(256)
gather_f32_k(const float* __restrict__ src, const int* __restrict__ idx, float* __restrict__ dst, long long n) {
    for (long long e = (long long)blockIdx.x * blockDim.x + threadIdx.x; e < n; e += (long long)gridDim.x * blockDim.x) {
        const int i = idx[e];
        dst[e] = i >= 0 ? src[i] : 0.f;
    }
}
}

extern "C" int vg_gather_f32(const float* src, const int32_t* idx, float* dst, int64_t n, void* stream) {
    if (!src || !idx || !dst || n <= 0) { vg_set_error("vg_gather_f32: bad arguments"); return VG_ERR_ARG; }
    long long blocks = (n + 255) / 256; if (blocks > 1024) blocks = 1024;
    vg_launch(gather_f32_k, dim3((unsigned)blocks), dim3(256), 0, (hipStream_t)stream, src, (const int*)idx, dst, (long long)n);
    return vg_check_launch("gather_f32");
}
```

vae-gam_amd/ops.py:

```python
import ctypes
from dataclasses import dataclass
from typing import Optional, Tuple

import torch

from . import _lib
from ._lib import ConvDesc, WgradDesc

BN_EPS = 1e-5

PROFILE = None
_LABEL = ['']


class label:
    def __init__(self, name):
        self.name = name

    def __enter__(self):
        self.prev = _LABEL[0]; _LABEL[0] = self.name

    def __exit__(self, *a):
        _LABEL[0] = self.prev


def _call(t, fn, *args):
    lib = _lib.get_lib()
    if not t.is_cuda and not lib.host_pointers_ok:
        raise RuntimeError('refusing to launch %s on a non-GPU tensor: the HIP kernels need device pointers (no CPU path)' % fn)
    if PROFILE is not None and t.is_cuda:
        e0 = torch.cuda.Event(enable_timing=True); e1 = torch.cuda.Event(enable_timing=True)
        e0.record()
        lib.call(fn, *args, _stream(t))
        e1.record()
        PROFILE.setdefault('%s:%s' % (fn, _LABEL[0]), []).append((e0, e1))
    else:
        lib.call(fn, *args, _stream(t))


import os as _os
SIDE_STREAM = bool(int(_os.environ.get('VG_SIDE_STREAM', '1')))
FUSE_LAST_BN_BWD = bool(int(_os.environ.get('VG_FUSE_LAST_BN_BWD', '1')))
WGRAD_BN_SUMS = bool(int(_os.environ.get('VG_WGRAD_BN_SUMS', '1')))
FC_SIDE_STREAM = bool(int(_os.environ.get('VG_FC_SIDE_STREAM', '0')))
_SIDE = {}


def _side_stream(device):
    key = (device.type, device.index)
    if key not in _SIDE:
        _SIDE[key] = torch.cuda.Stream(device=device)
    return _SIDE[key]


class on_side_stream:
    def __init__(self, ref, *tensors, enabled=None):
        self.active = bool((SIDE_STREAM if enabled is None else enabled) and ref.is_cuda)
        self.ref, self.tensors = ref, tensors

    def __enter__(self):
        if not self.active:
            return self
        self.side = _side_stream(self.ref.device)
        self.side.wait_stream(torch.cuda.current_stream(self.ref.device))
        _queue_join(self.ref.device)
        for t in self.tensors:
            if t is not None:
                t.record_stream(self.side)
        self.ctx = torch.cuda.stream(self.side)
        self.ctx.__enter__()
        return self

    def __exit__(self, *a):
        if self.active:
            self.ctx.__exit__(*a)


_JOIN_QUEUED = set()


def _queue_join(device):
    key = (device.type, device.index)
    if key in _JOIN_QUEUED:
        return
    _JOIN_QUEUED.add(key)

    def _cb():
        _JOIN_QUEUED.discard(key)
        join_side_stream(device)
    try:
        torch.autograd.Variable._execution_engine.queue_callback(_cb)
    except RuntimeError:
        _JOIN_QUEUED.discard(key)


def join_side_stream(device):
    key = (device.type, device.index)
    if key in _SIDE:
        torch.cuda.current_stream(device).wait_stream(_SIDE[key])


def _p(t):
    return None if t is None else ctypes.c_void_p(t.data_ptr())


def _stream(t):
    if t.is_cuda:
        return ctypes.c_void_p(torch.cuda.current_stream(t.device).cuda_stream)
    return None


def _chk(t, dtype=torch.float32):
    assert t.is_contiguous(), 'tensor must be contiguous'
    assert t.dtype == dtype, 'expected %s, got %s' % (dtype, t.dtype)
    return t


@dataclass(frozen=True)
class ConvSpec:
    kind: str
    ci: int
    co: int
    k: Tuple[int, int, int]
    stride: int
    pad: Tuple[int, int, int] = (0, 0, 0)
    outpad: Tuple[int, int, int] = (0, 0, 0)
    name: str = ''

    def out_size(self, i):
        if self.kind == 'conv':
            return tuple((i[a] + 2 * self.pad[a] - self.k[a]) // self.stride + 1 for a in range(3))
        return tuple((i[a] - 1) * self.stride - 2 * self.pad[a] + self.k[a] + self.outpad[a] for a in range(3))


def pack_weight(w: torch.Tensor, spec: ConvSpec, direction: str) -> torch.Tensor:
    fwd = direction == 'fwd'
    if (spec.kind == 'conv') == fwd:
        return w.permute(1, 2, 3, 4, 0).contiguous()
    if spec.stride == 1:
        w = w.flip(2, 3, 4)
    return w.permute(0, 2, 3, 4, 1).contiguous()


def pack_mode(spec: ConvSpec, direction: str) -> int:
    if (spec.kind == 'conv') == (direction == 'fwd'):
        return 0
    return 2 if spec.stride == 1 else 1


class PackedWeights:

    def __init__(self, layers, flat, offsets, sizes=None):
        self.mm = {}
        self._mm_idx = None
        if sizes is not None and USE_MM:
            import numpy as np
            idx_all, spans, pos = [], {}, 0
            for name, spec, w in layers:
                isz, osz = sizes[name]
                for direction in ('fwd', 'bwd'):
                    if direction == 'bwd' and name == 'conv1':
                        continue
                    plan = mm_plan(spec, 'fwd', isz) if direction == 'fwd' else mm_plan(spec, 'bwd', osz, isz)
                    if plan is None:
                        continue
                    gi = np.where(plan.aidx >= 0, plan.aidx + offsets[name], -1).astype(np.int32)
                    idx_all.append(gi); spans[(name, direction)] = (plan, pos, gi.size); pos += gi.size
            if idx_all:
                self._mm_idx = torch.from_numpy(np.concatenate(idx_all)).to(flat.device)
                self._mm_buf = torch.zeros(pos, dtype=torch.float32, device=flat.device)
                self.mm = {k: (plan, self._mm_buf[o:o + n]) for k, (plan, o, n) in spans.items()}
        segs, views, dst = [], {}, 0
        for name, spec, w in layers:
            for direction in ('fwd', 'bwd'):
                d0, d1 = w.shape[0], w.shape[1]
                kvol = w[0, 0].numel()
                n = w.numel()
                segs.append([offsets[name], dst, d0, d1, kvol, pack_mode(spec, direction), n, 0])
                views[(name, direction)] = (dst, n, pack_weight(w.detach(), spec, direction).shape)
                dst += ((n + 3) // 4) * 4
        self.total = dst
        self.flat = flat
        self.buf = torch.empty(dst, dtype=torch.float32, device=flat.device)
        self.segs = torch.tensor(segs, dtype=torch.int64).to(flat.device)
        self.nseg = len(segs)
        self._views = {k: self.buf[o:o + n].view(shape) for k, (o, n, shape) in views.items()}
        self.elems = dst

    def refresh(self):
        _call(self.flat, 'vg_pack_weights', _p(self.flat), _p(self.buf), _p(self.segs), self.nseg, self.elems)
        if self._mm_idx is not None:
            _call(self.flat, 'vg_gather_f32', _p(self.flat), _p(self._mm_idx), _p(self._mm_buf), self._mm_idx.numel())

    def get_mm(self, name, direction):
        return self.mm.get((name, direction))

    def get(self, name, direction):
        return self._views[(name, direction)]


def _conv_desc(N, ci, co, isz, osz, k, stride, pad, relu_in, per_group):
    return ConvDesc(N, ci, co, isz[0], isz[1], isz[2], osz[0], osz[1], osz[2], k[0], k[1], k[2], stride,
                    pad[0], pad[1], pad[2], int(relu_in), int(per_group))


def conv_forward(x, wpk, bias, spec: ConvSpec, relu_in=False, scale=None, shift=None, per_group=1, next_bn=None):
    lib = _lib.get_lib()
    N = x.shape[0]
    isz = tuple(x.shape[2:]); osz = spec.out_size(isz)
    y = torch.empty((N, spec.co) + osz, dtype=torch.float32, device=x.device)
    _chk(x); _chk(wpk)
    if spec.kind == 'conv':
        assert spec.pad == (0, 0, 0)
        d = _conv_desc(N, spec.ci, spec.co, isz, osz, spec.k, spec.stride, (0, 0, 0), relu_in, per_group)
        _call(x, 'vg_corr3d', ctypes.byref(d), _p(x), _p(wpk), _p(bias), _p(scale), _p(shift), None, _p(y))
    elif spec.stride == 1:
        padc = tuple(spec.k[a] - 1 - spec.pad[a] for a in range(3))
        d = _conv_desc(N, spec.ci, spec.co, isz, osz, spec.k, 1, padc, relu_in, per_group)
        _call(x, 'vg_corr3d', ctypes.byref(d), _p(x), _p(wpk), _p(bias), _p(scale), _p(shift), None, _p(y))
    else:
        d = _conv_desc(N, spec.ci, spec.co, isz, osz, spec.k, 2, spec.pad, relu_in, per_group)
        if next_bn:
            chunks = lib.size('vg_tconv3d_s2_stats_chunks', ctypes.byref(d), int(next_bn))
            G = N // int(next_bn)
            part = torch.empty(G * spec.co * chunks * 2, dtype=torch.float64, device=x.device)
            _call(x, 'vg_tconv3d_s2_stats', ctypes.byref(d), _p(x), _p(wpk), _p(bias), _p(scale), _p(shift), _p(y), int(next_bn), 1,
                     _p(part))
            return y, part
        else:
            _call(x, 'vg_tconv3d_s2', ctypes.byref(d), _p(x), _p(wpk), _p(bias), _p(scale), _p(shift), None, _p(y))
    if next_bn:
        raise ValueError('next_bn: only the stride-2 transposed-conv kernel accumulates the next layer\'s statistics')
    return y


def conv_backward_data(dy, wpk_bwd, spec: ConvSpec, in_size, mask_src=None):
    lib = _lib.get_lib()
    N = dy.shape[0]
    osz = tuple(dy.shape[2:]); isz = tuple(in_size)
    dx = torch.empty((N, spec.ci) + isz, dtype=torch.float32, device=dy.device)
    _chk(dy); _chk(wpk_bwd)
    if spec.kind == 'convt':
        d = _conv_desc(N, spec.co, spec.ci, osz, isz, spec.k, spec.stride, spec.pad, False, 1)
        _call(dy, 'vg_corr3d', ctypes.byref(d), _p(dy), _p(wpk_bwd), None, None, None, _p(mask_src), _p(dx))
    elif spec.stride == 1:
        padc = tuple(spec.k[a] - 1 for a in range(3))
        d = _conv_desc(N, spec.co, spec.ci, osz, isz, spec.k, 1, padc, False, 1)
        _call(dy, 'vg_corr3d', ctypes.byref(d), _p(dy), _p(wpk_bwd), None, None, None, _p(mask_src), _p(dx))
    else:
        d = _conv_desc(N, spec.co, spec.ci, osz, isz, spec.k, 2, (0, 0, 0), False, 1)
        _call(dy, 'vg_tconv3d_s2', ctypes.byref(d), _p(dy), _p(wpk_bwd), None, None, None, _p(mask_src), _p(dx))
    return dx


def conv_weight_grad(x, dy, spec: ConvSpec, relu_in=False, scale=None, shift=None, per_group=1, out=None):
    lib = _lib.get_lib()
    N = x.shape[0]
    isz = tuple(x.shape[2:]); osz = tuple(dy.shape[2:])
    _chk(x); _chk(dy)
    if spec.kind == 'conv':
        d = WgradDesc(N, spec.co, spec.ci, *osz, *isz, *spec.k, spec.stride, 0, 0, 0, 1, int(relu_in), int(per_group))
        a, b = x, dy
        shape = (spec.co, spec.ci) + tuple(spec.k)
    else:
        d = WgradDesc(N, spec.ci, spec.co, *isz, *osz, *spec.k, spec.stride, *spec.pad, 0, int(relu_in), int(per_group))
        a, b = dy, x
        shape = (spec.ci, spec.co) + tuple(spec.k)
    nbytes = lib.size('vg_wgrad3d_ws_bytes', ctypes.byref(d))
    ws = torch.empty(max(nbytes // 4, 1), dtype=torch.float32, device=x.device)
    if out is not None:
        assert out.shape == shape and out.is_contiguous() and out.dtype == torch.float32
        _call(x, 'vg_wgrad3d', ctypes.byref(d), _p(a), _p(b), _p(scale), _p(shift), _p(ws), _p(out), 1)
        return None
    dw = torch.empty(shape, dtype=torch.float32, device=x.device)
    _call(x, 'vg_wgrad3d', ctypes.byref(d), _p(a), _p(b), _p(scale), _p(shift), _p(ws), _p(dw), 0)
    return dw


def _bn_ws(x, N, C, P, per_group):
    nbytes = _lib.get_lib().size('vg_bn_ws_bytes', N, C, P, per_group)
    return torch.empty(nbytes // 8, dtype=torch.float64, device=x.device)


def bn_stats(x, gamma, beta, relu, per_group, sync=None, pre=None):
    lib = _lib.get_lib()
    N, C = x.shape[0], x.shape[1]
    P = x[0, 0].numel()
    G = N // per_group
    out = torch.empty((4, G * C), dtype=torch.float32, device=x.device)
    if pre is not None:
        assert relu, 'producer-side partials are statistics of relu(x)'
        part = pre
        assert part.dtype == torch.float64 and part.device == x.device and part.numel() % (G * C * 2) == 0
        chunks = part.numel() // (G * C * 2)
        sums = torch.empty((G * C, 3), dtype=torch.float64, device=x.device)
        count = float(per_group * P)
        if sync is None:
            _call(x, 'vg_bn_stats_from_parts', _p(part), G, C, chunks, count, _p(gamma), _p(beta), BN_EPS, None, _p(sums),
                     _p(out[0]), _p(out[1]), _p(out[2]), _p(out[3]))
        else:
            _call(x, 'vg_bn_stats_from_parts', _p(part), G, C, chunks, count, _p(gamma), _p(beta), BN_EPS, _p(sums), None,
                     None, None, None, None)
            sums = sync(sums)
            _call(x, 'vg_bn_finalize', _p(sums), G, C, _p(gamma), _p(beta), BN_EPS, _p(out[0]), _p(out[1]), _p(out[2]),
                     _p(out[3]))
        return out[0], out[1], out[2], out[3]
    ws = _bn_ws(x, N, C, P, per_group)
    if sync is None:
        _call(x, 'vg_bn_stats', _p(_chk(x)), N, C, P, per_group, int(relu), _p(gamma), _p(beta), BN_EPS, _p(ws), None,
                 _p(out[0]), _p(out[1]), _p(out[2]), _p(out[3]))
    else:
        sums = torch.empty((G * C, 3), dtype=torch.float64, device=x.device)
        _call(x, 'vg_bn_stats', _p(_chk(x)), N, C, P, per_group, int(relu), _p(gamma), _p(beta), BN_EPS, _p(ws), _p(sums),
                 None, None, None, None)
        sums = sync(sums)
        _call(x, 'vg_bn_finalize', _p(sums), G, C, _p(gamma), _p(beta), BN_EPS, _p(out[0]), _p(out[1]), _p(out[2]),
                 _p(out[3]))
    return out[0], out[1], out[2], out[3]


def _grad_buf(t):
    if isinstance(t, torch.nn.Parameter) and t.grad is not None and t.grad.is_contiguous() and t.grad.dtype == torch.float32:
        return t.grad
    return None


def bn_backward_(dxe, p, gamma, mean, rstd, relu, per_group, sync=None, beta=None, producer_bias_grad=None):
    lib = _lib.get_lib()
    N, C = p.shape[0], p.shape[1]
    P = p[0, 0].numel()
    G = N // per_group
    ws = _bn_ws(p, N, C, P, per_group)
    sums = torch.empty((G * C, 2), dtype=torch.float64, device=p.device)
    _call(p, 'vg_bn_bwd_reduce', _p(_chk(dxe)), _p(_chk(p)), N, C, P, per_group, int(relu), _p(mean), _p(rstd), _p(ws),
             _p(sums))
    count = float(per_group * P)
    local = None
    if sync is not None:
        local = sums.clone()
        sums = sync(sums)
        count = count * sync.world_size
    parts = torch.empty((2, G, C), dtype=torch.float32, device=p.device)
    if producer_bias_grad is not None:
        assert producer_bias_grad.shape == (C,) and producer_bias_grad.is_contiguous() and producer_bias_grad.dtype == torch.float32
    _call(p, 'vg_bn_bwd_apply', _p(dxe), _p(p), N, C, P, per_group, int(relu), _p(gamma), _p(mean), _p(rstd), _p(sums),
             count, _p(parts[0]), _p(parts[1]), _p(ws), _p(producer_bias_grad), 1)
    src = local if local is not None else sums
    gg, bg = _grad_buf(gamma), _grad_buf(beta)
    if gg is not None and bg is not None:
        _call(p, 'vg_bn_param_grad', _p(src), G, C, _p(gg), _p(bg), 1)
        return None, None
    dg = torch.empty(C, dtype=torch.float32, device=p.device); db = torch.empty_like(dg)
    _call(p, 'vg_bn_param_grad', _p(src), G, C, _p(dg), _p(db), 0)
    return dg, db


_GROUPED_OK = {}


def _grouped_wgrad_ok(p_shape, per_group):
    key = (tuple(p_shape), int(per_group))
    if key not in _GROUPED_OK:
        N, C, ID, IH, IW = key[0]
        d = WgradDesc(N, C, 1, ID, IH, IW, ID + 2, IH + 2, IW + 2, 3, 3, 3, 1, 0, 0, 0, 0, 0, int(per_group))
        _GROUPED_OK[key] = _lib.get_lib().dll.vg_wgrad3d_grouped_ws_bytes(ctypes.byref(d)) >= 0
    return _GROUPED_OK[key]


def bn_backward_tconv1(dy, weight, p, gamma, mean, rstd, relu, per_group, sync=None, beta=None, producer_bias_grad=None, dw_out=None):
    lib = _lib.get_lib()
    N, C = p.shape[0], p.shape[1]
    ID, IH, IW = p.shape[2:]
    assert tuple(dy.shape) == (N, 1, ID + 2, IH + 2, IW + 2) and tuple(weight.shape) == (C, 1, 3, 3, 3)
    _chk(dy); _chk(p)
    w = _chk(weight.detach().contiguous())
    G = N // per_group
    P = ID * IH * IW
    ws = torch.empty(lib.size('vg_bn_tconv1_ws_bytes', N, C, ID, per_group) // 8, dtype=torch.float64, device=p.device)
    sums = torch.empty((G * C, 2), dtype=torch.float64, device=p.device)
    if dw_out is not None:
        assert dw_out.shape == weight.shape and dw_out.is_contiguous() and dw_out.dtype == torch.float32 and beta is not None
        d = WgradDesc(N, C, 1, ID, IH, IW, ID + 2, IH + 2, IW + 2, 3, 3, 3, 1, 0, 0, 0, 0, int(relu), int(per_group))
        nbytes = lib.size('vg_wgrad3d_grouped_ws_bytes', ctypes.byref(d))
        wws = torch.empty(nbytes // 4, dtype=torch.float32, device=p.device)
        q = torch.empty((G, C + 1, 27), dtype=torch.float32, device=p.device)
        nshift = -(mean * rstd)
        _call(p, 'vg_wgrad3d_grouped', ctypes.byref(d), _p(dy), _p(p), _p(rstd), _p(nshift), _p(wws), _p(q))
        _call(p, 'vg_bn_tconv1_sums', _p(q), _p(w), _p(gamma), _p(beta), G, C, 27, _p(sums), _p(dw_out), 1)
    else:
        _call(p, 'vg_bn_bwd_reduce_tconv1', _p(dy), _p(w), _p(p), N, C, ID, IH, IW, per_group, int(relu), _p(mean), _p(rstd), _p(ws), _p(sums))
    count = float(per_group * P)
    local = None
    if sync is not None:
        local = sums.clone()
        sums = sync(sums)
        count = count * sync.world_size
    dp = torch.empty_like(p)
    if producer_bias_grad is not None:
        assert producer_bias_grad.shape == (C,) and producer_bias_grad.is_contiguous() and producer_bias_grad.dtype == torch.float32
    _call(p, 'vg_bn_bwd_apply_tconv1', _p(dy), _p(w), _p(p), _p(dp), N, C, ID, IH, IW, per_group, int(relu), _p(gamma), _p(mean), _p(rstd),
          _p(sums), count, _p(ws), _p(producer_bias_grad), 1)
    src = local if local is not None else sums
    gg, bg = _grad_buf(gamma), _grad_buf(beta)
    if gg is not None and bg is not None:
        _call(p, 'vg_bn_param_grad', _p(src), G, C, _p(gg), _p(bg), 1)
        return dp, None, None
    dg = torch.empty(C, dtype=torch.float32, device=p.device); db = torch.empty_like(dg)
    _call(p, 'vg_bn_param_grad', _p(src), G, C, _p(dg), _p(db), 0)
    return dp, dg, db


def channel_sum(x, out=None):
    lib = _lib.get_lib()
    N, C = x.shape[0], x.shape[1]
    P = x[0, 0].numel()
    ws = _bn_ws(x, N, C, P, N)
    if out is not None:
        assert out.shape == (C,) and out.is_contiguous() and out.dtype == torch.float32
        _call(x, 'vg_channel_sum', _p(_chk(x)), N, C, P, _p(ws), _p(out), 1)
        return None
    out = torch.empty(C, dtype=torch.float32, device=x.device)
    _call(x, 'vg_channel_sum', _p(_chk(x)), N, C, P, _p(ws), _p(out), 0)
    return out


class BnConvAct(torch.autograd.Function):

    @staticmethod
    def forward(ctx, p_in, weight, bias, gamma, beta, spec: ConvSpec, relu_in: bool, per_group: int,
                input_is_data: bool, sync, packed=None, next_bn=None, pre_stats=None, producer_bias=None,
                bias_grad_by_consumer=False):
        p_in = p_in.contiguous()
        has_bn = gamma is not None
        assert producer_bias is None or has_bn, 'producer_bias: the hand-off happens in the batch-norm backward'
        scale = shift = mean = rstd = None
        part = None
        with label(spec.name + '/fwd'):
            if has_bn:
                scale, shift, mean, rstd = bn_stats(p_in, gamma, beta, relu_in, per_group, sync, pre_stats)
            mmf = _mm_for(packed, weight, spec, 'fwd', tuple(p_in.shape[2:]), None)
            if mmf is not None:
                y = conv_mm(p_in, mmf[0], mmf[1], bias, relu_in, scale, shift, per_group, None, next_bn)
            else:
                wf = packed.get(spec.name, 'fwd') if packed is not None else pack_weight(weight, spec, 'fwd')
                y = conv_forward(p_in, wf, bias, spec, relu_in, scale, shift, per_group, next_bn)
            if next_bn:
                y, part = y
        ctx.spec, ctx.relu_in, ctx.per_group, ctx.input_is_data, ctx.sync, ctx.has_bn = \
            spec, relu_in, per_group, input_is_data, sync, has_bn
        ctx.save_for_backward(p_in, weight, gamma, beta, scale, shift, mean, rstd)
        ctx.bias_ref = bias
        ctx.packed = packed
        ctx.producer_bias, ctx.bias_grad_by_consumer = producer_bias, bool(bias_grad_by_consumer)
        ctx.nout = 2 if next_bn else 1
        if next_bn:
            ctx.mark_non_differentiable(part)
            return y, part
        return y

    @staticmethod
    def backward(ctx, dy, *_unused):
        with label(ctx.spec.name + '/bwd'):
            return BnConvAct._backward(ctx, dy) + (None, None, None)

    @staticmethod
    def _backward(ctx, dy):
        p_in, weight, gamma, beta, scale, shift, mean, rstd = ctx.saved_tensors
        spec, relu_in, per_group = ctx.spec, ctx.relu_in, ctx.per_group
        dy = dy.contiguous()
        wg = weight.grad if (isinstance(weight, torch.nn.Parameter) and weight.grad is not None and weight.grad.is_contiguous()) else None
        bias_t = ctx.bias_ref
        bg = bias_t.grad if (isinstance(bias_t, torch.nn.Parameter) and bias_t.grad is not None and bias_t.grad.is_contiguous()) else None
        direct_db = bg is not None and not (ctx.input_is_data and ctx.has_bn)
        overlap = direct_db and wg is not None and not ctx.input_is_data
        skip_db = ctx.bias_grad_by_consumer
        fuse_last = FUSE_LAST_BN_BWD and ctx.has_bn and not ctx.input_is_data and spec.kind == 'convt' and spec.stride == 1 \
            and spec.co == 1 and tuple(spec.k) == (3, 3, 3) and tuple(spec.pad) == (0, 0, 0) and spec.ci <= 16
        dw_by_bn = fuse_last and WGRAD_BN_SUMS and _grouped_wgrad_ok(p_in.shape, per_group)
        if dw_by_bn:
            overlap = False
        if overlap:
            with on_side_stream(dy, dy, p_in, scale, shift, wg, bg):
                if not skip_db:
                    channel_sum(dy, out=bg)
                conv_weight_grad(p_in, dy, spec, relu_in, scale, shift, per_group, out=wg)
            db = dw = None
        elif skip_db:
            db = None
        else:
            db = channel_sum(dy, out=bg) if direct_db else channel_sum(dy)
        dgamma = dbeta = dp = None
        if ctx.input_is_data:
            if ctx.has_bn:
                assert spec.kind == 'conv' and spec.pad == (0, 0, 0) and not relu_in
                G = p_in.shape[0] // per_group
                assert G == 1
                nshift = torch.empty_like(mean)
                _call(mean, 'vg_data_bn_nshift', _p(_chk(mean)), _p(_chk(rstd)), mean.numel(), _p(nshift))
                dw_hat = conv_weight_grad(p_in, dy, spec, False, rstd, nshift, per_group)
                gg, gbt = _grad_buf(gamma), _grad_buf(beta)
                acc = wg is not None and bg is not None and gg is not None and gbt is not None
                taps = spec.k[0] * spec.k[1] * spec.k[2]
                dw = wg if acc else torch.empty_like(weight)
                dbo = bg if acc else torch.empty_like(db)
                dgamma = gg if acc else torch.empty_like(gamma)
                dbeta = gbt if acc else torch.empty_like(beta)
                _call(dy, 'vg_data_bn_grads', _p(_chk(dw_hat)), _p(_chk(db)), _p(_chk(weight)), _p(_chk(gamma)), _p(_chk(beta)),
                      spec.co, spec.ci, taps, _p(dw), _p(dbo), _p(dgamma), _p(dbeta), int(acc))
                if acc:
                    return None, None, None, None, None, None, None, None, None, None, None, None
                db = dbo
            else:
                dw = conv_weight_grad(p_in, dy, spec, relu_in, None, None, per_group, out=wg)
            return None, dw, db, dgamma, dbeta, None, None, None, None, None, None, None
        if dw_by_bn:
            dw = None
        elif not overlap:
            dw = conv_weight_grad(p_in, dy, spec, relu_in, scale, shift, per_group, out=wg)
        in_size = tuple(p_in.shape[2:])
        mmb = _mm_for(ctx.packed, weight, spec, 'bwd', tuple(dy.shape[2:]), in_size)
        wb = None
        if mmb is None:
            wb = ctx.packed.get(spec.name, 'bwd') if ctx.packed is not None else pack_weight(weight, spec, 'bwd')
        if ctx.has_bn:
            pbg = None
            if ctx.producer_bias is not None:
                pb = ctx.producer_bias
                if pb.grad is None:
                    raise RuntimeError('bn_conv_act: producer_bias.grad is not bound -- the consumer adds the producer\'s bias gradient into it '
                                       '(FusedAdam binds every .grad to its flat buffer; a free-standing caller sets .grad = zeros first)')
                pbg = pb.grad
            if fuse_last:
                dw_t = (wg if wg is not None else torch.zeros_like(weight)) if dw_by_bn else None
                dp, dgamma, dbeta = bn_backward_tconv1(dy, weight, p_in, gamma, mean, rstd, relu_in, per_group, ctx.sync, beta, pbg, dw_out=dw_t)
                if dw_by_bn and wg is None:
                    dw = dw_t
            else:
                dp = conv_mm(dy, mmb[0], mmb[1], None, False, None, None, 1, None) if mmb is not None else \
                    conv_backward_data(dy, wb, spec, in_size, None)
                dgamma, dbeta = bn_backward_(dp, p_in, gamma, mean, rstd, relu_in, per_group, ctx.sync, beta, pbg)
        else:
            msk = p_in if relu_in else None
            dp = conv_mm(dy, mmb[0], mmb[1], None, False, None, None, 1, msk) if mmb is not None else \
                conv_backward_data(dy, wb, spec, in_size, msk)
        return dp, dw, db, dgamma, dbeta, None, None, None, None, None, None, None


_MM_SKIP = set(filter(None, _os.environ.get('VG_MM_SKIP', '').split(',')))


def mm_wins(plan):
    if plan is None:
        return False
    if _MM_SKIP and 'k%d' % plan.ks[0] in _MM_SKIP and (plan.PDT + plan.PD - 1) // plan.PD > 1:
        return False
    if USE_MM >= 2 or (plan.PDT + plan.PD - 1) // plan.PD == 1:
        return True
    if plan.mode == 'tconv':
        return list(plan.ks) in ([3, 2, 2, 1], [2, 1, 1, 1], [2, 2, 2, 2])
    return plan.ks[0] in (7, 9)


def _mm_for(packed, weight, spec, direction, read_size, write_size):
    if not USE_MM or (direction == 'bwd' and spec.co == 1):
        return None
    if packed is not None:
        got = packed.get_mm(spec.name, direction)
        if got is not None and (got[0].ID, got[0].IH, got[0].IW) == tuple(read_size):
            return got if mm_wins(got[0]) else None
    plan = mm_plan(spec, direction, read_size, write_size)
    if not mm_wins(plan):
        return None
    return plan, plan.gather(weight)


def bn_conv_act(p_in, weight, bias, gamma, beta, spec, relu_in, per_group=None, input_is_data=False, sync=None, packed=None,
                next_bn=None, pre_stats=None, producer_bias=None, bias_grad_by_consumer=False):
    if per_group is None:
        per_group = p_in.shape[0]
    return BnConvAct.apply(p_in, weight, bias, gamma, beta, spec, relu_in, per_group, input_is_data, sync, packed, next_bn,
                           pre_stats, producer_bias, bias_grad_by_consumer)


class GamElbo(torch.autograd.Function):

    @staticmethod
    def forward(ctx, logits, gain, x, eps, glm, logits_bias=None):
        lib = _lib.get_lib()
        G, B, V = logits.shape
        C = G - 1
        logits = _chk(logits.contiguous()); gain = _chk(gain.contiguous()); x = _chk(x.contiguous())
        eps = _chk(eps.contiguous(), torch.float64); glm = _chk(glm.contiguous())
        ws = torch.empty(lib.size('vg_gam_ws_bytes', C, B, V) // 4 + 1, dtype=torch.float32, device=x.device)
        slp = torch.empty(B, dtype=torch.float32, device=x.device)
        dist = torch.empty((C, B), dtype=torch.float32, device=x.device)
        _call(x, 'vg_gam_elbo_fwd', _p(logits), _p(gain), _p(x), _p(eps), _p(glm), C, B, V, _p(ws), _p(slp), _p(dist),
                 None)
        ctx.save_for_backward(logits, gain, x, eps, glm, dist)
        ctx.logits_bias = logits_bias
        return slp, dist

    @staticmethod
    def backward(ctx, g_slp, g_dist):
        lib = _lib.get_lib()
        logits, gain, x, eps, glm, dist = ctx.saved_tensors
        tot = None
        if ctx.logits_bias is not None:
            pb = ctx.logits_bias
            assert pb.numel() == 1
            if pb.grad is None:
                raise RuntimeError('GamElbo: logits_bias.grad is not bound (see bn_conv_act: the bias gradient is added into the caller\'s buffer)')
            tot = pb.grad
        G, B, V = logits.shape
        C = G - 1
        g_slp = _chk(g_slp.contiguous()); g_dist = _chk(g_dist.contiguous())
        ws = torch.empty(lib.size('vg_gam_ws_bytes', C, B, V) // 4 + 1, dtype=torch.float32, device=x.device)
        d_logits = torch.empty_like(logits)
        d_gain = torch.empty_like(gain)
        d_eps = torch.empty_like(eps)
        _call(x, 'vg_gam_elbo_bwd', _p(logits), _p(gain), _p(x), _p(eps), _p(glm), _p(dist), _p(g_slp), _p(g_dist),
                 C, B, V, _p(ws), _p(d_logits), _p(d_gain), _p(d_eps), _p(tot), 1)
        return d_logits, d_gain, None, d_eps, None, None


class LatentSample(torch.autograd.Function):

    @staticmethod
    def forward(ctx, mu, w, a, eps_w, eps_d, G):
        B, L = mu.shape
        mu = _chk(mu.contiguous()); w = _chk(w.contiguous()); a = _chk(a.contiguous())
        eps_w = _chk(eps_w.contiguous()); eps_d = _chk(eps_d.contiguous())
        assert w.shape == (B, L) and a.shape == (B, L) and eps_d.shape == (B, L) and eps_w.numel() == B
        zcat = torch.empty((G * B, L + G), dtype=torch.float32, device=mu.device)
        kl = torch.empty(B, dtype=torch.float32, device=mu.device)
        d = torch.empty((B, L), dtype=torch.float32, device=mu.device)
        flag = torch.empty(1, dtype=torch.float32, device=mu.device)
        _call(mu, 'vg_latent_fwd', _p(mu), _p(w), _p(a), _p(eps_w), _p(eps_d), B, L, G, _p(zcat), _p(kl), _p(d), _p(flag))
        ctx.save_for_backward(mu, w, d, flag, eps_w, eps_d)
        ctx.G = G
        ctx.mark_non_differentiable(d)
        return zcat, kl, d

    @staticmethod
    def backward(ctx, g_zcat, g_kl, _g_d):
        mu, w, d, flag, eps_w, eps_d = ctx.saved_tensors
        B, L = mu.shape
        g_mu = torch.empty_like(mu); g_w = torch.empty_like(mu); g_a = torch.empty_like(mu)
        gz = _p(_chk(g_zcat.contiguous())) if g_zcat is not None else None
        gk = _p(_chk(g_kl.contiguous())) if g_kl is not None else None
        _call(mu, 'vg_latent_bwd', _p(mu), _p(w), _p(d), _p(flag), _p(eps_w), _p(eps_d), gz, gk, B, L, ctx.G,
                 _p(g_mu), _p(g_w), _p(g_a))
        return g_mu, g_w, g_a, None, None, None


class LatentSampleStacked(torch.autograd.Function):

    @staticmethod
    def forward(ctx, mwa, eps_w, eps_d, G):
        mwa = _chk(mwa.contiguous())
        _, B, L = mwa.shape
        eps_w = _chk(eps_w.contiguous()); eps_d = _chk(eps_d.contiguous())
        assert eps_d.shape == (B, L) and eps_w.numel() == B
        zcat = torch.empty((G * B, L + G), dtype=torch.float32, device=mwa.device)
        kl = torch.empty(B, dtype=torch.float32, device=mwa.device)
        d = torch.empty((B, L), dtype=torch.float32, device=mwa.device)
        flag = torch.empty(1, dtype=torch.float32, device=mwa.device)
        _call(mwa, 'vg_latent_fwd', _p(mwa[0]), _p(mwa[1]), _p(mwa[2]), _p(eps_w), _p(eps_d), B, L, G, _p(zcat), _p(kl), _p(d), _p(flag))
        ctx.save_for_backward(mwa, d, flag, eps_w, eps_d)
        ctx.G = G
        ctx.mark_non_differentiable(d)
        return zcat, kl, d

    @staticmethod
    def backward(ctx, g_zcat, g_kl, _g_d):
        mwa, d, flag, eps_w, eps_d = ctx.saved_tensors
        _, B, L = mwa.shape
        g = torch.empty_like(mwa)
        gz = _p(_chk(g_zcat.contiguous())) if g_zcat is not None else None
        gk = _p(_chk(g_kl.contiguous())) if g_kl is not None else None
        _call(mwa, 'vg_latent_bwd', _p(mwa[0]), _p(mwa[1]), _p(d), _p(flag), _p(eps_w), _p(eps_d), gz, gk, B, L, ctx.G,
                 _p(g[0]), _p(g[1]), _p(g[2]))
        return g, None, None, None


class ElboLoss(torch.autograd.Function):

    @staticmethod
    def forward(ctx, kl_z, slp, dist, gp_kl, coef):
        kl_z = _chk(kl_z.contiguous()); slp = _chk(slp.contiguous()); dist = _chk(dist.contiguous()); gp_kl = _chk(gp_kl.contiguous())
        loss = torch.empty(1, dtype=torch.float32, device=kl_z.device)
        ctx.coef = tuple(float(c) for c in coef)
        ctx.shapes = (kl_z.shape, slp.shape, dist.shape, gp_kl.shape)
        _call(kl_z, 'vg_loss_fwd', _p(kl_z), _p(slp), _p(dist), _p(gp_kl), kl_z.numel(), dist.numel(), *ctx.coef, _p(loss))
        return loss

    @staticmethod
    def backward(ctx, g):
        sk, ss, sd, sg = ctx.shapes
        g = _chk(g.contiguous())
        g_kl = torch.empty(sk, dtype=torch.float32, device=g.device); g_slp = torch.empty(ss, dtype=torch.float32, device=g.device)
        g_dist = torch.empty(sd, dtype=torch.float32, device=g.device); g_gp = torch.empty(sg, dtype=torch.float32, device=g.device)
        _call(g, 'vg_loss_bwd', _p(g), g_kl.numel(), g_dist.numel(), *ctx.coef, _p(g_kl), _p(g_slp), _p(g_dist), _p(g_gp))
        return g_kl, g_slp, g_dist, g_gp, None


def _fc_split(M, N, K):
    tiles = ((M + 31) // 32) * ((N + 31) // 32)
    if K <= 1024:
        return 1
    ks = max(1, min(K // 256, 1024 // tiles))
    if ks <= 1:
        return 1
    kchunk = (((K + ks - 1) // ks) + 63) // 64 * 64
    return (K + kchunk - 1) // kchunk


def fc_job(A, B, C, M, N, K, a_strides, b_strides, c_strides, flags=0, batch=1, bias=None, bias_sb=0, amask=None, cmask=None,
           cx=None, cx_sb=0, ksplit=None):
    lib = _lib.get_lib()
    if ksplit is None:
        ksplit = _fc_split(M, N + (1 if flags & _lib.FC_B_ONES else 0), K) if batch == 1 else 1
    d = _lib.FcDesc(M, N, K, batch, a_strides[0], a_strides[1], a_strides[2], b_strides[0], b_strides[1], b_strides[2],
                    c_strides[0], c_strides[1], bias_sb, cx_sb, ksplit, flags)
    ws = None
    if ksplit > 1:
        ws = torch.empty(lib.size('vg_fc_ws_bytes', ctypes.byref(d)) // 4, dtype=torch.float32, device=C.device)
    ptr = lambda t: None if t is None else t.data_ptr()
    return _lib.FcJob(d, ptr(A), ptr(amask), ptr(B), ptr(bias), ptr(cmask), ptr(C), ptr(cx), ptr(ws)), (A, B, C, bias, amask, cmask, cx, ws)


def fc_launch(ref, jobs):
    arr = (_lib.FcJob * len(jobs))(*[j[0] for j in jobs])
    _call(ref, 'vg_fc_gemm_jobs', arr, len(jobs))


def fc_gemm(A, B, C, *args, **kw):
    fc_launch(C, [fc_job(A, B, C, *args, **kw)])
    return C


def _fc_forward(x, weight, bias, relu, relu_in):
    M, K = x.shape; N = weight.shape[0]
    y = torch.empty((M, N), dtype=torch.float32, device=x.device)
    fl = _lib.FC_C_BIAS | (_lib.FC_C_RELU if relu else 0) | (_lib.FC_A_RELU if relu_in else 0)
    return fc_gemm(x, weight, y, M, N, K, (x.stride(0), 1, 0), (1, weight.stride(0), 0), (N, 0), fl, bias=bias)


def _fc_backward(gy, x, weight, y, relu_in, need_gx, wg, bg):
    M, N = gy.shape; K = x.shape[1]
    am = _lib.FC_A_MASK if y is not None else 0
    jobs = []
    gx = None
    if need_gx:
        gx = torch.empty((M, K), dtype=torch.float32, device=gy.device)
        jobs.append(fc_job(gy, weight, gx, M, K, N, (N, 1, 0), (weight.stride(0), 1, 0), (K, 0), am | (_lib.FC_C_MASK if relu_in else 0),
                           amask=y, cmask=x if relu_in else None))
    acc = wg is not None and bg is not None
    gw = wg if acc else torch.empty((N, K), dtype=torch.float32, device=gy.device)
    gb = bg if acc else torch.empty((N,), dtype=torch.float32, device=gy.device)
    jobs.append(fc_job(gy, x, gw, N, K, M, (1, N, 0), (x.stride(0), 1, 0), (K, 0),
                       am | _lib.FC_B_ONES | (_lib.FC_B_RELU if relu_in else 0) | (_lib.FC_C_ACCUM if acc else 0), amask=y, cx=gb))
    fc_launch(gy, jobs)
    return gx, (None if acc else gw), (None if acc else gb)


class LinearAct(torch.autograd.Function):

    @staticmethod
    def forward(ctx, x, weight, bias, relu, relu_in=False):
        x = _chk(x.contiguous()); _chk(weight); _chk(bias)
        y = _fc_forward(x, weight, bias, relu, relu_in)
        ctx.relu, ctx.relu_in = relu, relu_in
        ctx.save_for_backward(x, weight, y if relu else None)
        ctx.bias_ref = bias
        return y

    @staticmethod
    def backward(ctx, gy):
        x, weight, y = ctx.saved_tensors
        bias = ctx.bias_ref
        gy = _chk(gy.contiguous())
        gx, gw, gb = _fc_backward(gy, x, weight, y, ctx.relu_in, ctx.needs_input_grad[0], _grad_buf(weight), _grad_buf(bias))
        return gx, gw, gb, None, None


class HeadsAct(torch.autograd.Function):

    @staticmethod
    def forward(ctx, h, W3, b3, W4, b4, gW3, gb3, gW4, gb4):
        B = h.shape[0]
        h = _chk(h.contiguous())
        G, L, H = W4.shape
        y = _fc_forward(h, W3, b3, True, False)
        out = torch.empty((G, B, L), dtype=torch.float32, device=h.device)
        fc_gemm(y, W4, out, B, L, H, (G * H, 1, H), (1, H, L * H), (L, B * L), _lib.FC_C_BIAS, batch=G, bias=b4, bias_sb=L)
        ctx.save_for_backward(h, y, W3, W4)
        ctx.grads = (gW3, gb3, gW4, gb4)
        return out

    @staticmethod
    def backward(ctx, gout):
        h, y, W3, W4 = ctx.saved_tensors
        gW3, gb3, gW4, gb4 = ctx.grads
        B = h.shape[0]
        G, L, H = W4.shape
        gout = _chk(gout.contiguous())
        gX = torch.empty((B, G * H), dtype=torch.float32, device=h.device)
        fc_launch(gout, [fc_job(gout, W4, gX, B, H, L, (L, 1, B * L), (H, 1, L * H), (G * H, H), 0, batch=G),
                         fc_job(gout, y, gW4, L, H, B, (1, L, B * L), (G * H, 1, H), (H, L * H), _lib.FC_B_ONES | _lib.FC_C_ACCUM, batch=G,
                                cx=gb4, cx_sb=L)])
        gh, _, _ = _fc_backward(gX, h, W3, y, False, True, gW3, gb3)
        return gh, None, None, None, None, None, None, None, None


_ONES = {}


def _ones(n, device):
    key = (n, str(device))
    if key not in _ONES:
        _ONES[key] = torch.ones(n, dtype=torch.float32, device=device)
    return _ONES[key]


def linear_act(layer, x, relu, relu_in=False):
    return LinearAct.apply(x, layer.weight, layer.bias, relu, relu_in)


def gam_maps(logits, gain, x, eps, glm):
    lib = _lib.get_lib()
    G, B, V = logits.shape
    C = G - 1
    ws = torch.empty(lib.size('vg_gam_ws_bytes', C, B, V) // 4 + 1, dtype=torch.float32, device=x.device)
    slp = torch.empty(B, dtype=torch.float32, device=x.device)
    dist = torch.empty((max(C, 1), B), dtype=torch.float32, device=x.device)
    maps = torch.empty((G + 1, B, V), dtype=torch.float32, device=x.device)
    _call(x, 'vg_gam_elbo_fwd', _p(_chk(logits.contiguous())), _p(_chk(gain.contiguous())), _p(_chk(x.contiguous())),
             _p(_chk(eps.contiguous(), torch.float64)), _p(_chk(glm.contiguous())), C, B, V, _p(ws), _p(slp), _p(dist),
             _p(maps))
    return maps


class CholeskyF64(torch.autograd.Function):

    @staticmethod
    def forward(ctx, a):
        assert a.dtype == torch.float64 and a.dim() == 3 and a.shape[1] == a.shape[2]
        a = a.contiguous()
        l = torch.empty_like(a)
        _call(a, 'vg_cholesky_f64', _p(a), _p(l), a.shape[0], a.shape[1])
        ctx.save_for_backward(l)
        return l

    @staticmethod
    def backward(ctx, gl):
        (l,) = ctx.saved_tensors
        p = (l.transpose(1, 2) @ gl).tril()
        p = p - 0.5 * torch.diag_embed(p.diagonal(dim1=1, dim2=2))
        x = torch.linalg.solve_triangular(l.transpose(1, 2), p, upper=True)
        s = torch.linalg.solve_triangular(l, x, upper=False, left=False)
        return 0.5 * (s + s.transpose(1, 2))


def cholesky(a):
    if a.dtype == torch.float64 and a.shape[-1] <= 128 and (a.is_cuda or _lib.get_lib().host_pointers_ok):
        return CholeskyF64.apply(a)
    return torch.linalg.cholesky_ex(a, check_errors=False).L


GAIN_MAX_BATCH = 4096
GAIN_FORCE_TILED = False


def check_gain_batch(B, what='the gain block'):
    if int(B) > GAIN_MAX_BATCH:
        raise ValueError('%s would draw the gains of %d volumes jointly: the limit is %d volumes per joint draw (vg_gp_gain_fwd). '
                         'Use a smaller minibatch or, under data parallelism, dp_gain=\'local\' (each rank draws its own slice).'
                         % (what, int(B), GAIN_MAX_BATCH))


class GainConsts:

    def __init__(self, table, xu, hrf, n, jitter_ku=0.0, jitter_b=1e-5, prior_var=10.0):
        self.table, self.xu, self.hrf = table, xu, hrf
        self.C, self.n = int(table.shape[0]), int(n)
        self.jitter_ku, self.jitter_b, self.prior_var = float(jitter_ku), float(jitter_b), float(prior_var)

    def desc(self, B):
        return _lib.GainDesc(self.C, int(B), self.n, int(self.hrf.numel()), self.jitter_b, self.jitter_ku, self.prior_var)


class GpGain(torch.autograd.Function):

    @staticmethod
    def forward(ctx, covariates, eps_beta, consts, flat_p, flat_g, join_stream, *params):
        lib = _lib.get_lib()
        B = covariates.shape[0]
        C = consts.C
        assert covariates.dtype == torch.float32 and covariates.dim() == 2 and covariates.shape[1] >= C and covariates.stride(1) == 1
        eps_beta = _chk(eps_beta.contiguous())
        assert eps_beta.shape == (C, B)
        dev = covariates.device
        d = consts.desc(B)
        ws = torch.empty(lib.size('vg_gp_gain_ws_bytes', C, B, consts.n) // 8, dtype=torch.float64, device=dev)
        tv = torch.empty((C, B), dtype=torch.float32, device=dev)
        kl = torch.empty(1, dtype=torch.float32, device=dev)
        bm = torch.empty((C, B), dtype=torch.float64, device=dev)
        bc = torch.empty((C, B, B), dtype=torch.float64, device=dev)
        fb = torch.zeros((C, B), dtype=torch.float64, device=dev)
        sg = torch.zeros((C, B, B), dtype=torch.float64, device=dev)
        tiled = bool(GAIN_FORCE_TILED)
        _call(covariates, 'vg_gp_gain_fwd_tiled' if tiled else 'vg_gp_gain_fwd', ctypes.byref(d), _p(consts.table), _p(flat_p), _p(consts.xu), _p(covariates),
              int(covariates.stride(0)), _p(eps_beta), _p(consts.hrf), _p(ws), _p(tv), _p(kl), _p(bm), _p(bc), _p(fb), _p(sg))
        kl_terms = ws[-(C + 8):-8]
        ctx.save_for_backward(covariates, eps_beta, ws)
        ctx.consts, ctx.flat_p, ctx.flat_g, ctx.join_stream, ctx.tiled = consts, flat_p, flat_g, join_stream, tiled
        ctx.mark_non_differentiable(bm, bc, fb, sg, kl_terms)
        return tv, kl, bm, bc, fb, sg, kl_terms

    @staticmethod
    def backward(ctx, g_tv, g_kl, *_):
        covariates, eps_beta, ws = ctx.saved_tensors
        consts = ctx.consts
        B = covariates.shape[0]
        d = consts.desc(B)
        if g_tv is None:
            g_tv = torch.zeros((consts.C, B), dtype=torch.float32, device=covariates.device)
        if g_kl is None:
            g_kl = torch.zeros(1, dtype=torch.float32, device=covariates.device)
        g_tv = _chk(g_tv.contiguous()); g_kl = _chk(g_kl.contiguous())
        _call(covariates, 'vg_gp_gain_bwd_tiled' if ctx.tiled else 'vg_gp_gain_bwd', ctypes.byref(d), _p(consts.table), _p(ctx.flat_p), _p(consts.xu), _p(covariates),
              int(covariates.stride(0)), _p(eps_beta), _p(consts.hrf), _p(ws), _p(g_tv), _p(g_kl), _p(ctx.flat_g))
        if ctx.join_stream is not None and covariates.is_cuda:
            cur = torch.cuda.current_stream(covariates.device)
            if cur != ctx.join_stream:
                ctx.join_stream.wait_stream(cur)
        return (None,) * len(ctx.needs_input_grad)


class HrfAcrossRanks(torch.autograd.Function):

    @staticmethod
    def forward(ctx, pre, T, dp, lo):
        B = pre.shape[1]
        full = dp.all_gather_rows(pre.t().contiguous()).t()
        ctx.save_for_backward(T)
        ctx.dp, ctx.lo, ctx.B = dp, int(lo), int(B)
        return (full @ T)[:, lo:lo + B].contiguous()

    @staticmethod
    def backward(ctx, g):
        (T,) = ctx.saved_tensors
        lo, B = ctx.lo, ctx.B
        gp = g.contiguous() @ T[:, lo:lo + B].t()
        gp = ctx.dp.allreduce_sum_(gp)
        return gp[:, lo:lo + B].contiguous(), None, None, None


def adam_advance_(state, lr, b1, b2):
    _call(state, 'vg_adam_advance', _p(_chk(state, torch.float64)), float(lr), float(b1), float(b2))


def adam_step_(p, g, m, v, b1, b2, eps, step_scalars):
    lib = _lib.get_lib()
    assert p.dtype == g.dtype == m.dtype == v.dtype and p.dtype in (torch.float32, torch.float64)
    assert p.is_contiguous() and g.is_contiguous() and m.is_contiguous() and v.is_contiguous()
    _call(p, 'vg_adam_step', _p(p), _p(g), _p(m), _p(v), p.numel(), int(p.dtype == torch.float64), float(b1), float(b2),
             float(eps), _p(_chk(step_scalars, torch.float64)))


GUARD_STATE_LEN = _lib.GUARD_STATE_LEN
GUARD_NORM, GUARD_SCALE, GUARD_APPLY, GUARD_SEEN, GUARD_SKIPPED, GUARD_CLIPPED, GUARD_NORM_SUM, GUARD_NORM_MAX = range(8)


def grad_guard_ws(g32, g64):
    ref = g32 if g32 is not None else g64
    n = _lib.get_lib().size('vg_grad_guard_ws_bytes', 0 if g32 is None else g32.numel(), 0 if g64 is None else g64.numel())
    return torch.empty(n // 8, dtype=torch.float64, device=ref.device)


def grad_guard_(g32, g64, max_norm, skip_nonfinite, ws, state):
    ref = g32 if g32 is not None else g64
    if g32 is not None:
        _chk(g32, torch.float32)
    if g64 is not None:
        _chk(g64, torch.float64)
    assert state.numel() == GUARD_STATE_LEN
    _call(ref, 'vg_grad_guard', _p(g32), 0 if g32 is None else g32.numel(), _p(g64), 0 if g64 is None else g64.numel(),
          float(max_norm) if max_norm else 0.0, int(bool(skip_nonfinite)), _p(_chk(ws, torch.float64)), _p(_chk(state, torch.float64)))


def adam_advance_guarded_(state, lr, b1, b2, guard):
    _call(state, 'vg_adam_advance_guarded', _p(_chk(state, torch.float64)), float(lr), float(b1), float(b2),
          _p(_chk(guard, torch.float64)))


def adam_step_guarded_(p, g, m, v, b1, b2, eps, step_scalars, guard):
    assert p.dtype == g.dtype == m.dtype == v.dtype and p.dtype in (torch.float32, torch.float64)
    assert p.is_contiguous() and g.is_contiguous() and m.is_contiguous() and v.is_contiguous()
    _call(p, 'vg_adam_step_guarded', _p(p), _p(g), _p(m), _p(v), p.numel(), int(p.dtype == torch.float64), float(b1), float(b2),
          float(eps), _p(_chk(step_scalars, torch.float64)), _p(_chk(guard, torch.float64)))


USE_MM = int(_os.environ.get('VG_CONV_MM', '1'))
_MM_LDS_BUDGET = 150 * 1024
_MM_LDS_CU = 160 * 1024
_MM_TUNED = {
    ('corr', 1, 16, 16, (3, 3, 3), (6, 8, 5), (8, 10, 7)): (8, 4, 10, 16, 0),
    ('corr', 1, 16, 16, (3, 3, 3), (8, 10, 7), (6, 8, 5)): (8, 3, 8, 16, 0),
    ('corr', 2, 16, 16, (3, 3, 3), (16, 21, 14), (8, 10, 7)): (8, 2, 10, 8, 0),
    ('corr', 1, 16, 8, (3, 3, 3), (17, 21, 14), (19, 23, 16)): (8, 1, 23, 8, 0),
    ('corr', 1, 8, 16, (3, 3, 3), (19, 23, 16), (17, 21, 14)): (8, 1, 21, 8, 0),
    ('corr', 1, 8, 16, (3, 3, 3), (18, 23, 16), (16, 21, 14)): (8, 2, 11, 8, 1),
    ('tconv', 2, 8, 8, (5, 3, 3), (18, 23, 16), (39, 47, 33)): (8, 2, 12, 8, 1),
}
_MM_WAVES = 8


class MmPlan:

    def __init__(self, **kw):
        self.__dict__.update(kw)
        self._dev = {}

    def tables(self, device):
        key = str(device)
        if key not in self._dev:
            self._dev[key] = (torch.from_numpy(self.tau).to(device), torch.from_numpy(self.dlt).to(device), torch.from_numpy(self.aidx).to(device))
        return self._dev[key]

    def desc(self, N, relu_in, per_group):
        d = _lib.MmDesc()
        for k in ('CI', 'CO', 'ID', 'IH', 'IW', 'OD', 'OH', 'OW', 'nq', 'PDT', 'PH', 'PW', 'PD', 'sdi', 'shi', 'swi', 'd0', 'LD', 'cc', 'sdo', 'sho',
                  'swo', 'tpc', 'slack', 'dbuf', 'PHB', 'hlo', 'hhi', 'waves'):
            setattr(d, k, int(getattr(self, k)))
        d.N, d.relu_in, d.per_group = int(N), int(bool(relu_in)), int(per_group)
        for q in range(4):
            d.ks[q] = int(self.ks[q]) if q < self.nq else 0
            d.od0[q] = int(self.od0[q]) if q < self.nq else 0
            d.oh0[q] = int(self.oh0[q]) if q < self.nq else 0
            d.ow0[q] = int(self.ow0[q]) if q < self.nq else 0
        return d

    def gather(self, weight):
        _, _, aidx = self.tables(weight.device)
        flat = weight.detach().reshape(-1)
        a = flat[aidx.clamp_min(0).long()]
        return torch.where(aidx >= 0, a, torch.zeros_like(a)).contiguous()


def _mm_problem(spec: ConvSpec, direction: str, in_size):
    import numpy as np
    KD, KH, KW = spec.k
    kvol = KD * KH * KW
    conv = spec.kind == 'conv'

    def w_at(ci_layer, co_layer, kd, kh, kw):
        t = (kd * KH + kh) * KW + kw
        return ((co_layer * spec.ci + ci_layer) if conv else (ci_layer * spec.co + co_layer)) * kvol + t
    fl = lambda kd, kh, kw: (KD - 1 - kd, KH - 1 - kh, KW - 1 - kw)
    if direction == 'fwd':
        osz = spec.out_size(in_size)
        if conv:
            return 'corr', spec.stride, (0, 0, 0), spec.ci, spec.co, spec.k, osz, (lambda cin, kd, kh, kw, cout: w_at(cin, cout, kd, kh, kw))
        if spec.stride == 1:
            pad = tuple(spec.k[a] - 1 - spec.pad[a] for a in range(3))
            return 'corr', 1, pad, spec.ci, spec.co, spec.k, osz, (lambda cin, kd, kh, kw, cout: w_at(cin, cout, *fl(kd, kh, kw)))
        return 'tconv', 2, tuple(spec.pad), spec.ci, spec.co, spec.k, osz, (lambda cin, kd, kh, kw, cout: w_at(cin, cout, kd, kh, kw))
    if conv:
        isz = None
        if spec.stride == 1:
            pad = tuple(spec.k[a] - 1 for a in range(3))
            return 'corr', 1, pad, spec.co, spec.ci, spec.k, isz, (lambda cin, kd, kh, kw, cout: w_at(cout, cin, *fl(kd, kh, kw)))
        return 'tconv', 2, (0, 0, 0), spec.co, spec.ci, spec.k, isz, (lambda cin, kd, kh, kw, cout: w_at(cout, cin, kd, kh, kw))
    return 'corr', spec.stride, tuple(spec.pad), spec.co, spec.ci, spec.k, None, (lambda cin, kd, kh, kw, cout: w_at(cout, cin, kd, kh, kw))


_MM_PLANS = {}


def mm_plan(spec: ConvSpec, direction: str, in_size, out_size=None, force=None) -> Optional[MmPlan]:
    import numpy as np
    key = (spec, direction, tuple(in_size), None if out_size is None else tuple(out_size), force)
    if key in _MM_PLANS:
        return _MM_PLANS[key]
    mode, S, pad, CI, CO, K, osz, widx = _mm_problem(spec, direction, tuple(in_size))
    if osz is None:
        osz = tuple(out_size)
    plan = None
    if CO in (8, 16) and CI >= 8 and not (mode == 'tconv' and CO != 8):
        plan = _mm_build(mode, S, pad, CI, CO, K, tuple(in_size), tuple(osz), widx, force)
    _MM_PLANS[key] = plan
    return plan


def _mm_build(mode, S, pad, CI, CO, K, isz, osz, widx, force=None):
    import numpy as np
    KD, KH, KW = K
    ID, IH, IW = isz
    OD, OH, OW = osz
    IHW = IH * IW
    NR = 16 // CO
    classes = []
    if mode == 'corr':
        KWp = KW + (NR - 1) * S
        ent = []
        for kd in range(KD):
            for kh in range(KH):
                for kwp in range(KWp):
                    def tap(rho, kd=kd, kh=kh, kwp=kwp):
                        kw = kwp - rho * S
                        return (kd, kh, kw) if 0 <= kw < KW else None
                    ent.append((kd - pad[0], kh - pad[1], kwp - pad[2], tap))
        classes.append(ent)
        PDT, PH, PW = OD, OH, (OW + NR - 1) // NR
        sdi, shi, swi = S, S, NR * S
        sdo, sho, swo = 1, 1, NR
        od0, oh0, ow0 = [0], [0], [0]
        d0 = -pad[0]
        ld_of = lambda PD: (PD - 1) * S + KD
    else:
        assert NR == 2 and S == 2
        MDm = (KD + 1) // 2
        od0, oh0, ow0 = [], [], []
        for rd, rh in ((0, 0), (0, 1), (1, 0), (1, 1)):
            if True:
                ent = []
                for md in range((KD - rd + 1) // 2):
                    for mh in range((KH - rh + 1) // 2):
                        for mw in range(2):
                            def tap(rho, rd=rd, rh=rh, md=md, mh=mh, mw=mw):
                                kw = rho + 2 * mw
                                return (rd + 2 * md, rh + 2 * mh, kw) if kw < KW else None
                            ent.append((-md, -mh, -mw, tap))
                classes.append(ent)
                od0.append(rd - pad[0]); oh0.append(rh - pad[1]); ow0.append(-pad[2])
        PDT, PH, PW = (OD + pad[0] + 1) // 2, (OH + pad[1] + 1) // 2, (OW + pad[2] + 1) // 2
        sdi = shi = swi = 1
        sdo = sho = swo = 2
        d0 = -(MDm - 1)
        ld_of = lambda PD: PD + MDm - 1
    nq = len(classes)
    if nq not in (1, 4) or any(len(e) == 0 for e in classes):
        return None
    ks = [(len(e) + 3) // 4 for e in classes]
    if max(ks) > 32:
        return None
    rows = sum(ks)
    tau = np.zeros((rows, 4), np.int32); dlt = np.zeros((rows, 4, 3), np.int32)
    aidx = []
    slack = 0
    r0 = 0
    for q, ent in enumerate(classes):
        a = -np.ones((CI, ks[q], 64), np.int32)
        for s in range(ks[q]):
            for kk in range(4):
                kap = 4 * s + kk
                e = ent[kap] if kap < len(ent) else ent[0]
                dd, dh, dw = e[0], e[1], e[2]
                tau[r0 + s, kk] = dd * IHW + dh * IW + dw
                dlt[r0 + s, kk] = (dd, dh, dw)
                slack = max(slack, abs(dh) * IW + abs(dw) + 1)
                if kap >= len(ent):
                    continue
                for row in range(16):
                    rho, co = row // CO, row % CO
                    t = e[3](rho)
                    if t is None:
                        continue
                    lane = kk * 16 + row
                    for ci in range(CI):
                        a[ci, s, lane] = widx(ci, t[0], t[1], t[2], co)
        aidx.append(a.reshape(-1))
        r0 += ks[q]
    aidx = np.concatenate(aidx)
    tpc_max = (8 if max(ks) <= 12 else 3) if nq == 1 else 4
    hlo, hhi = int(dlt[:, :, 1].min()), int(dlt[:, :, 1].max())
    tuned = _MM_TUNED.get((mode, S, CI, CO, tuple(K), tuple(isz), tuple(osz))) if force is None else None
    pin = force or tuned
    cands = []
    for W in (8, 4):
        for PD in range(min(PDT, 16), 0, -1):
            LD = ld_of(PD)
            for nslab in (1, 2, 3, 4, 6, 8, 12):
                PHB = (PH + nslab - 1) // nslab
                if nslab > 1 and ((PH + PHB - 1) // PHB != nslab or PHB < 2):
                    continue
                npos = PD * PHB * PW
                tpc = (npos + W * 16 - 1) // (W * 16)
                if tpc > tpc_max:
                    continue
                rows_max = min((PHB - 1) * shi + (hhi - hlo) + 1, IH)
                whole = (nslab == 1 and hlo <= 0 and (PH - 1) * shi + hhi + 1 >= IH)
                LPH = IHW if whole else ((rows_max * IW + 3) // 4) * 4 + 4
                CHP = 64 + ((LD * LPH + 63) // 64) * 64
                bps = ((PDT + PD - 1) // PD) * nslab
                for cc in ([CI] if nq > 1 else [c for c in range(CI, 0, -1) if CI % c == 0]):
                    for dbuf in (1, 0):
                        if pin and (W, PD, PHB, cc, dbuf) != tuple(pin):
                            continue
                        lds = (((aidx.size + 63) // 64) * 64 + rows * 64 + (1 + dbuf) * cc * CHP + 64) * 4
                        if lds > _MM_LDS_BUDGET:
                            continue
                        per_simd = 4 if (tpc <= 3 or nq > 1) else 2
                        nblk = min(_MM_LDS_CU // lds, per_simd * 4 // W)
                        if nblk < 1:
                            continue
                        util = npos / float(tpc * W * 16) * (PDT / float(((PDT + PD - 1) // PD) * PD)) * (PH / float(nslab * PHB))
                        halo = ((PD * sdi) / float(LD)) * min(1.0, (PHB * shi) / float(rows_max))
                        wps = nblk * W // 4
                        occ = {1: 0.45, 2: 0.6, 3: 0.8}.get(wps, 1.0)
                        shape = (1.0 if nslab == 1 else 0.85) * (1.0 if W == 8 else 0.9)
                        score = util * (0.5 + 0.5 * halo) * (0.9 + 0.1 * cc / float(CI)) * occ * shape * (1.0 if (dbuf or nblk >= 2) else 0.9)
                        cands.append((score, PD, LD, cc, tpc, dbuf, PHB, W))
    if not cands:
        return None
    _, PD, LD, cc, tpc, dbuf, PHB, W = max(cands, key=lambda c: (round(c[0], 9), c[3], -c[5]))
    tpc = {1: (3 if tpc <= 3 else tpc if tpc <= 6 else 8), 4: 4}[nq]
    return MmPlan(CI=CI, CO=CO, ID=ID, IH=IH, IW=IW, OD=OD, OH=OH, OW=OW, nq=nq, ks=ks, PDT=PDT, PH=PH, PW=PW, PD=PD, sdi=sdi, shi=shi,
                  swi=swi, d0=d0, LD=LD, cc=cc, sdo=sdo, sho=sho, swo=swo, od0=od0, oh0=oh0, ow0=ow0, tpc=tpc, slack=slack, dbuf=dbuf,
                  PHB=PHB, hlo=hlo, hhi=hhi, waves=W,
                  tau=tau.reshape(-1), dlt=dlt.reshape(-1), aidx=aidx, mode=mode)


def conv_mm(x, plan: MmPlan, aimg, bias, relu_in, scale, shift, per_group, mask_src=None, next_bn=None):
    lib = _lib.get_lib()
    N = x.shape[0]
    assert tuple(x.shape[1:]) == (plan.CI, plan.ID, plan.IH, plan.IW), (tuple(x.shape), plan.CI, plan.ID, plan.IH, plan.IW)
    tau, dlt, _ = plan.tables(x.device)
    d = plan.desc(N, relu_in, per_group if scale is not None else 1)
    y = torch.empty((N, plan.CO, plan.OD, plan.OH, plan.OW), dtype=torch.float32, device=x.device)
    _chk(x); _chk(aimg)
    if next_bn:
        chunks = lib.size('vg_conv_mm_stats_chunks', ctypes.byref(d), int(next_bn))
        G = N // int(next_bn)
        part = torch.zeros(G * plan.CO * chunks * 2, dtype=torch.float64, device=x.device)
        _call(x, 'vg_conv_mm', ctypes.byref(d), _p(x), _p(aimg), _p(tau), _p(dlt), _p(bias), _p(scale), _p(shift), _p(mask_src), _p(y),
              int(next_bn), 1, _p(part))
        return y, part
    _call(x, 'vg_conv_mm', ctypes.byref(d), _p(x), _p(aimg), _p(tau), _p(dlt), _p(bias), _p(scale), _p(shift), _p(mask_src), _p(y), 1, 0, None)
    return y
```

Baseline: 10020 volumes/s.

## Fuse BN backward reductions into data-grad conv_mm epilogue and merge tail kernels

The data-gradient implicit-GEMM conv now computes the batch-norm backward partial sums (sum of dy and sum of dy*x_hat) in its epilogue, using the BN mean/rstd and the pre-activation tensor loaded as a mask source. A new apply kernel folds those per-chunk partials itself, so the separate bn_bwd_reduce pass over dp and p goes away. The csum fold and the dgamma/dbeta reduction are merged into one tail launch. In exchange the conv epilogue gains extra loads and FMAs, and a new template instance (MASKED==2) handles only certain plans (nq=1, ks 7/9, tpc<=3).

```diff
diff --git a/include/vaegam.h b/include/vaegam.h
--- a/include/vaegam.h
+++ b/include/vaegam.h
@@ -42,8 +42,11 @@
     int32_t PHB;
     int32_t hlo, hhi;
     int32_t waves;
+    const float* bn_mean;
+    const float* bn_rstd;
 } vg_mm_desc;
 int64_t vg_conv_mm_stats_chunks(const vg_mm_desc* d, int32_t stats_per_group);
+int32_t vg_conv_mm_bnsums_ok(const vg_mm_desc* d);
 int vg_conv_mm(const vg_mm_desc* d, const float* x, const float* a_img, const int32_t* tau, const int32_t* dlt, const float* bias,
                const float* in_scale, const float* in_shift, const float* mask_src, float* y, int32_t stats_per_group,
                int32_t stats_relu, double* stats_part, void* stream);
@@ -84,6 +87,11 @@
                     int32_t relu, const float* gamma, const float* mean, const float* rstd,
                     const double* sums, double count, float* dgamma_part, float* dbeta_part,
                     void* ws, float* chsum, int32_t chsum_accumulate, void* stream);
+
+int vg_bn_bwd_apply_parts(float* dxe_inout, const float* p, int32_t N, int32_t C, int64_t P, int32_t per_group, int32_t relu,
+                          const float* gamma, const float* mean, const float* rstd, const double* part, int64_t part_chunks,
+                          double count, double* sums, void* ws, float* chsum, int32_t chsum_accumulate,
+                          float* dgamma, float* dbeta, int32_t accumulate, void* stream);
 
 int64_t vg_bn_tconv1_ws_bytes(int32_t N, int32_t C, int32_t ID, int32_t per_group);
 int vg_bn_bwd_reduce_tconv1(const float* dy, const float* w, const float* p, int32_t N, int32_t C, int32_t ID, int32_t IH, int32_t IW,
diff --git a/vae-gam_amd/_lib.py b/vae-gam_amd/_lib.py
--- a/vae-gam_amd/_lib.py
+++ b/vae-gam_amd/_lib.py
@@ -22,7 +22,8 @@
 class MmDesc(ctypes.Structure):
     _fields_ = [(n, i32) for n in ('N', 'CI', 'CO', 'ID', 'IH', 'IW', 'OD', 'OH', 'OW', 'nq')] + [('ks', i32 * 4)] + \
                [(n, i32) for n in ('PDT', 'PH', 'PW', 'PD', 'sdi', 'shi', 'swi', 'd0', 'LD', 'cc', 'sdo', 'sho', 'swo')] + \
-               [('od0', i32 * 4), ('oh0', i32 * 4), ('ow0', i32 * 4)] + [(n, i32) for n in ('relu_in', 'per_group', 'tpc', 'slack', 'dbuf', 'PHB', 'hlo', 'hhi', 'waves')]
+               [('od0', i32 * 4), ('oh0', i32 * 4), ('ow0', i32 * 4)] + [(n, i32) for n in ('relu_in', 'per_group', 'tpc', 'slack', 'dbuf', 'PHB', 'hlo', 'hhi', 'waves')] + \
+               [('bn_mean', vp), ('bn_rstd', vp)]
 
 
 class GainDesc(ctypes.Structure):
@@ -60,6 +61,7 @@
     'vg_bn_finalize': (ctypes.c_int, [vp, i32, i32, vp, vp, f32, vp, vp, vp, vp, vp]),
     'vg_bn_bwd_reduce': (ctypes.c_int, [vp, vp, i32, i32, i64, i32, i32, vp, vp, vp, vp, vp]),
     'vg_bn_bwd_apply': (ctypes.c_int, [vp, vp, i32, i32, i64, i32, i32, vp, vp, vp, vp, f64, vp, vp, vp, vp, i32, vp]),
+    'vg_bn_bwd_apply_parts': (ctypes.c_int, [vp, vp, i32, i32, i64, i32, i32, vp, vp, vp, vp, i64, f64, vp, vp, vp, i32, vp, vp, i32, vp]),
     'vg_bn_tconv1_ws_bytes': (i64, [i32, i32, i32, i32]),
     'vg_bn_bwd_reduce_tconv1': (ctypes.c_int, [vp, vp, vp, i32, i32, i32, i32, i32, i32, i32, vp, vp, vp, vp, vp]),
     'vg_bn_bwd_apply_tconv1': (ctypes.c_int, [vp, vp, vp, vp, i32, i32, i32, i32, i32, i32, i32, vp, vp, vp, vp, f64, vp, vp, i32, vp]),
@@ -81,6 +83,7 @@
     'vg_pack_weights': (ctypes.c_int, [vp, vp, vp, i32, i64, vp]),
     'vg_cholesky_f64': (ctypes.c_int, [vp, vp, i32, i32, vp]),
     'vg_conv_mm_stats_chunks': (i64, [ctypes.POINTER(MmDesc), i32]),
+    'vg_conv_mm_bnsums_ok': (i32, [ctypes.POINTER(MmDesc)]),
     'vg_conv_mm': (ctypes.c_int, [ctypes.POINTER(MmDesc), vp, vp, vp, vp, vp, vp, vp, vp, vp, i32, i32, vp, vp]),
     'vg_gather_f32': (ctypes.c_int, [vp, vp, vp, i64, vp]),
     'vg_fc_ws_bytes': (i64, [ctypes.POINTER(FcDesc)]),
diff --git a/vae-gam_amd/csrc/vg_bn.hip b/vae-gam_amd/csrc/vg_bn.hip
--- a/vae-gam_amd/csrc/vg_bn.hip
+++ b/vae-gam_amd/csrc/vg_bn.hip
@@ -109,20 +109,36 @@
     }
 }
 
+template <bool PARTS>
 __global__ void __launch_bounds__(BN_THREADS)
 bn_bwd_apply_k(float* __restrict__ dxe, const float* __restrict__ p, int C, long long P, int per_group, int relu,
                const float* __restrict__ gamma, const float* __restrict__ mean, const float* __restrict__ rstd,
-               const double* __restrict__ sums, double count, int cp, float* __restrict__ dgamma_part, float* __restrict__ dbeta_part,
-               double* __restrict__ csum_part) {
+               const double* __restrict__ sums, int pchunks, double* __restrict__ sums_out, double count, int cp,
+               float* __restrict__ dgamma_part, float* __restrict__ dbeta_part, double* __restrict__ csum_part) {
     const int chunk = blockIdx.x, c = blockIdx.y, g = blockIdx.z, chunks = gridDim.x;
     const int cpi = chunk % cp, si = chunk / cp, ns = chunks / cp;
     const int gc = g * C + c;
     const float mu = mean[gc], rs = rstd[gc];
-    const float m1 = (float)(sums[(size_t)gc * 2] / count), m2 = (float)(sums[(size_t)gc * 2 + 1] / count);
+    double s0, s1;
+    if (PARTS) {
+        __shared__ double folded[2];
+        double a = 0, b = 0;
+        for (int k = threadIdx.x; k < pchunks; k += BN_THREADS) { a += sums[((size_t)gc * pchunks + k) * 2]; b += sums[((size_t)gc * pchunks + k) * 2 + 1]; }
+        block_sum2(a, b);
+        if (threadIdx.x == 0) {
+            folded[0] = a; folded[1] = b;
+            if (chunk == 0) { sums_out[(size_t)gc * 2] = a; sums_out[(size_t)gc * 2 + 1] = b; }
+        }
+        __syncthreads();
+        s0 = folded[0]; s1 = folded[1];
+    } else {
+        s0 = sums[(size_t)gc * 2]; s1 = sums[(size_t)gc * 2 + 1];
+    }
+    const float m1 = (float)(s0 / count), m2 = (float)(s1 / count);
     const float k = (gamma ? gamma[c] : 1.f) * rs;
-    if (chunk == 0 && threadIdx.x == 0) {
-        dbeta_part[gc] = (float)sums[(size_t)gc * 2];
-        dgamma_part[gc] = (float)sums[(size_t)gc * 2 + 1];
+    if (!PARTS && chunk == 0 && threadIdx.x == 0) {
+        dbeta_part[gc] = (float)s0;
+        dgamma_part[gc] = (float)s1;
     }
     float vs = 0.f;
     for (int nn = si; nn < per_group; nn += ns) {
@@ -145,14 +161,35 @@
     }
 }
 
-__global__ void __launch_bounds__(BN_THREADS)
-csum_fold_k(const double* __restrict__ part, int G, int C, int chunks, int accumulate, float* __restrict__ out) {
-    const int c = blockIdx.x, lane = threadIdx.x;
+__device__ __forceinline__ void csum_fold_job(const double* __restrict__ part, int G, int C, int chunks, int accumulate,
+                                              float* __restrict__ out, int c) {
+    const int lane = threadIdx.x;
     double a = 0, unused = 0;
     for (int g = 0; g < G; ++g)
         for (int k = lane; k < chunks; k += BN_THREADS) a += part[((size_t)g * C + c) * chunks + k];
     block_sum2(a, unused);
     if (lane == 0) out[c] = (accumulate ? out[c] : 0.f) + (float)a;
+}
+
+__global__ void __launch_bounds__(BN_THREADS)
+csum_fold_k(const double* __restrict__ part, int G, int C, int chunks, int accumulate, float* __restrict__ out) {
+    csum_fold_job(part, G, C, chunks, accumulate, out, blockIdx.x);
+}
+
+__device__ __forceinline__ void bn_param_grad_job(const double* __restrict__ sums, int G, int C, int accumulate,
+                                                  float* __restrict__ dgamma, float* __restrict__ dbeta, int c) {
+    if (c >= C) return;
+    double a = 0, b = 0;
+    for (int g = 0; g < G; ++g) { b += sums[((size_t)g * C + c) * 2]; a += sums[((size_t)g * C + c) * 2 + 1]; }
+    dgamma[c] = (accumulate ? dgamma[c] : 0.f) + (float)a;
+    dbeta[c] = (accumulate ? dbeta[c] : 0.f) + (float)b;
+}
+
+__global__ void __launch_bounds__(BN_THREADS)
+bn_bwd_tail_k(const double* __restrict__ csum_part, int nfold, int G, int C, int chunks, int chsum_accumulate, float* __restrict__ chsum,
+              const double* __restrict__ sums, int accumulate, float* __restrict__ dgamma, float* __restrict__ dbeta) {
+    if ((int)blockIdx.x < nfold) csum_fold_job(csum_part, G, C, chunks, chsum_accumulate, chsum, blockIdx.x);
+    else bn_param_grad_job(sums, G, C, accumulate, dgamma, dbeta, ((int)blockIdx.x - nfold) * BN_THREADS + (int)threadIdx.x);
 }
 
 struct BnPlan { int cp, ns; int chunks() const { return cp * ns; } };
@@ -249,8 +286,8 @@
     const int G = N / per_group;
     const BnPlan pl = plan_for(P, per_group, C, G);
     double* csum_part = chsum ? (double*)ws : nullptr;
-    vg_launch(bn_bwd_apply_k, dim3(pl.chunks(), C, G), dim3(BN_THREADS), 0, (hipStream_t)stream, dxe, p, (int)C, (long long)P,
-              (int)per_group, (int)relu, gamma, mean, rstd, sums, count, pl.cp, dgamma_part, dbeta_part, csum_part);
+    vg_launch(bn_bwd_apply_k<false>, dim3(pl.chunks(), C, G), dim3(BN_THREADS), 0, (hipStream_t)stream, dxe, p, (int)C, (long long)P,
+              (int)per_group, (int)relu, gamma, mean, rstd, sums, 0, (double*)nullptr, count, pl.cp, dgamma_part, dbeta_part, csum_part);
     if ((rc = vg_check_launch("bn_bwd_apply"))) return rc;
     if (chsum) {
         vg_launch(csum_fold_k, dim3(C), dim3(BN_THREADS), 0, (hipStream_t)stream, (const double*)csum_part, G, (int)C, pl.chunks(),
@@ -258,6 +295,29 @@
         return vg_check_launch("bn_bwd csum_fold");
     }
     return VG_OK;
+}
+
+extern "C" int vg_bn_bwd_apply_parts(float* dxe, const float* p, int32_t N, int32_t C, int64_t P, int32_t per_group, int32_t relu,
+                                     const float* gamma, const float* mean, const float* rstd, const double* part, int64_t part_chunks,
+                                     double count, double* sums, void* ws, float* chsum, int32_t chsum_accumulate,
+                                     float* dgamma, float* dbeta, int32_t accumulate, void* stream) {
+    int rc = bn_args_ok("vg_bn_bwd_apply_parts", dxe, N, C, P, per_group);
+    if (rc) return rc;
+    if (!p || !mean || !rstd || !part || part_chunks <= 0 || part_chunks > 0x7fffffff || !sums || !dgamma || !dbeta || !(count > 0)) {
+        vg_set_error("vg_bn_bwd_apply_parts: bad argument"); return VG_ERR_ARG;
+    }
+    if (chsum && !ws) { vg_set_error("vg_bn_bwd_apply_parts: chsum needs the vg_bn_ws_bytes workspace"); return VG_ERR_ARG; }
+    hipStream_t s = (hipStream_t)stream;
+    const int G = N / per_group;
+    const BnPlan pl = plan_for(P, per_group, C, G);
+    double* csum_part = chsum ? (double*)ws : nullptr;
+    vg_launch(bn_bwd_apply_k<true>, dim3(pl.chunks(), C, G), dim3(BN_THREADS), 0, s, dxe, p, (int)C, (long long)P, (int)per_group, (int)relu,
+              gamma, mean, rstd, part, (int)part_chunks, sums, count, pl.cp, (float*)nullptr, (float*)nullptr, csum_part);
+    if ((rc = vg_check_launch("bn_bwd_apply(parts)"))) return rc;
+    const int nfold = chsum ? C : 0;
+    vg_launch(bn_bwd_tail_k, dim3(nfold + vg_cdiv(C, BN_THREADS)), dim3(BN_THREADS), 0, s, (const double*)csum_part, nfold, G, (int)C, pl.chunks(),
+              (int)chsum_accumulate, chsum, (const double*)sums, (int)accumulate, dgamma, dbeta);
+    return vg_check_launch("bn_bwd_tail");
 }
 
 namespace {
@@ -556,12 +616,7 @@
 namespace {
 __global__ void __launch_bounds__(64)
 bn_param_grad_k(const double* __restrict__ sums, int G, int C, int accumulate, float* __restrict__ dgamma, float* __restrict__ dbeta) {
-    const int c = blockIdx.x * blockDim.x + threadIdx.x;
-    if (c >= C) return;
-    double a = 0, b = 0;
-    for (int g = 0; g < G; ++g) { b += sums[((size_t)g * C + c) * 2]; a += sums[((size_t)g * C + c) * 2 + 1]; }
-    dgamma[c] = (accumulate ? dgamma[c] : 0.f) + (float)a;
-    dbeta[c] = (accumulate ? dbeta[c] : 0.f) + (float)b;
+    bn_param_grad_job(sums, G, C, accumulate, dgamma, dbeta, blockIdx.x * blockDim.x + threadIdx.x);
 }
 __global__ void __launch_bounds__(256)
 data_bn_grads_k(const float* __restrict__ dw_hat, const float* __restrict__ db, const float* __restrict__ w,
diff --git a/vae-gam_amd/csrc/vg_conv_mm.hip b/vae-gam_amd/csrc/vg_conv_mm.hip
--- a/vae-gam_amd/csrc/vg_conv_mm.hip
+++ b/vae-gam_amd/csrc/vg_conv_mm.hip
@@ -43,7 +43,7 @@
     if constexpr (I < N) { f(mm_int<I>{}); mm_static_for<N, I + 1>(f); }
 }
 
-template <int MM_W, int NQ, int TPC, int K0, int K1, int K2, int K3, bool DB, int OCC, bool MASKED>
+template <int MM_W, int NQ, int TPC, int K0, int K1, int K2, int K3, bool DB, int OCC, int MASKED>
 __global__ void __launch_bounds__(MM_W * VG_WAVE, OCC)
 conv_mm_k(const float* __restrict__ x, const float* __restrict__ a_img, const int* __restrict__ tau, const int* __restrict__ dlt,
           const float* __restrict__ bias, const float* __restrict__ in_scale, const float* __restrict__ in_shift,
@@ -140,6 +140,7 @@
     vg_f32x4 acc[TPC];
     float st_s[4] = {0.f, 0.f, 0.f, 0.f}, st_q[4] = {0.f, 0.f, 0.f, 0.f};
     float mreg[MASKED ? TPC : 1][4];
+    float bn_mu[4], bn_rs[4];
     float bias_l[4];
 #pragma unroll
     for (int r = 0; r < 4; ++r) bias_l[r] = bias ? bias[co_l + r] : 0.f;
@@ -182,7 +183,7 @@
 #pragma unroll
             for (int r = 0; r < 4; ++r) {
                 float v = acc[i].v[r] + bias_l[r];
-                if constexpr (MASKED) {
+                if constexpr (MASKED == 1) {
                     if constexpr (NQ == 1) v = (mreg[i][r] > 0.f) ? v : 0.f;
                     else v = (*reinterpret_cast<const float*>(mn + (size_t)r * ovol * 4 + off) > 0.f) ? v : 0.f;
                 }
@@ -199,13 +200,17 @@
 #else
                 *reinterpret_cast<float*>(yn + (size_t)r * ovol * 4 + off) = v;
 #endif
-                if (stats_part) {
+                if constexpr (MASKED == 2) {
+                    const float h = stats_relu ? vg_max(mreg[i][r], 0.f) : mreg[i][r];
+                    st_s[r] += v; st_q[r] = fmaf(v, (h - bn_mu[r]) * bn_rs[r], st_q[r]);
+                } else if (stats_part) {
                     const float h = stats_relu ? vg_max(v, 0.f) : v;
                     st_s[r] += h; st_q[r] = fmaf(h, h, st_q[r]);
                 }
             }
         }
     };
+    int n_run0 = 0;
     auto flush_stats = [&](int n) __attribute__((always_inline)) {
         const int g = n / stats_pg;
         const size_t chunks = (size_t)stats_pg * p.bps * MM_W;
@@ -219,6 +224,12 @@
             if (jl == 0 && (CO == 16 || kk < 2)) {
                 double* dst = stats_part + (((size_t)g * CO + co_l + r) * chunks + chunkid) * 2;
                 dst[0] = (double)sa; dst[1] = (double)sb;
+                if constexpr (MASKED == 2) {
+                    for (int m = n - p.nsplit; m >= n_run0; m -= p.nsplit) {
+                        double* z = dst - (size_t)((n - m) * p.bps * MM_W) * 2;
+                        z[0] = 0.0; z[1] = 0.0;
+                    }
+                }
             }
             st_s[r] = 0.f; st_q[r] = 0.f;
         }
@@ -296,7 +307,7 @@
         __syncthreads();
         VG_STAMP_ADD(2);
         if (DB && u + 1 < units) stage(u + 1);
-        if constexpr (NQ == 1 && MASKED) { if (chunk == nchunks - 1) load_mask(n); }
+        if constexpr (NQ == 1 && MASKED != 0) { if (chunk == nchunks - 1) load_mask(n); }
         VG_STAMP_ADD(3);
         auto class_work = [&](auto qc, auto ntc) __attribute__((always_inline)) {
             constexpr int q = decltype(qc)::value;
@@ -356,6 +367,13 @@
         };
         const int g_now = stats_part ? n / stats_pg : 0;
         if (stats_part && chunk == 0 && g_run >= 0 && g_now != g_run) flush_stats(n_run);
+        if constexpr (MASKED == 2) {
+            if (chunk == 0 && g_now != g_run) {
+                n_run0 = n;
+#pragma unroll
+                for (int r = 0; r < 4; ++r) { bn_mu[r] = d.bn_mean[g_now * CO + co_l + r]; bn_rs[r] = d.bn_rstd[g_now * CO + co_l + r]; }
+            }
+        }
         if constexpr (NQ == 1) {
             if (chunk == 0) zero_acc();
             if (nact > 0) mm_dispatch<TPC>(nact, [&](auto ntc) __attribute__((always_inline)) { class_work(mm_int<0>{}, ntc); });
@@ -406,8 +424,6 @@
         vg_set_error("%s: bad descriptor", who); return VG_ERR_ARG;
     }
     p->d = *d;
-    int ns = 256 / p->bps; if (ns < 1) ns = 1; if (ns > d->N) ns = d->N;
-    p->nsplit = ns;
     int row = 0, af = 0;
     for (int q = 0; q < d->nq; ++q) {
         if (d->ks[q] <= 0 || d->ks[q] > 32) { vg_set_error("%s: k-steps per channel must be 1..32 (class %d: %d)", who, q, d->ks[q]); return VG_ERR_ARG; }
@@ -433,6 +449,8 @@
     p->tau_off = ((p->aimg_floats + 63) / 64) * 64;
     p->in_off = p->tau_off + p->kstot * 64;
     p->bps = vg_cdiv(d->PDT, d->PD) * p->nhb;
+    int ns = 256 / p->bps; if (ns < 1) ns = 1; if (ns > d->N) ns = d->N;
+    p->nsplit = ns;
     const size_t total = (size_t)p->in_off + (d->dbuf ? 2 : 1) * (size_t)p->buf_floats + 64;
     *shmem = total * sizeof(float);
     if (*shmem > 160 * 1024) { vg_set_error("%s: plan needs %zu bytes of LDS", who, *shmem); return VG_ERR_UNSUPPORTED; }
@@ -444,6 +462,10 @@
     if (!d || stats_per_group <= 0 || d->PD <= 0 || d->PDT <= 0 || d->PH <= 0 || (d->waves != 4 && d->waves != 8)) return -1;
     const int PHB = (d->PHB > 0 && d->PHB < d->PH) ? d->PHB : d->PH;
     return (int64_t)stats_per_group * vg_cdiv(d->PDT, d->PD) * vg_cdiv(d->PH, PHB) * d->waves;
+}
+
+extern "C" int32_t vg_conv_mm_bnsums_ok(const vg_mm_desc* d) {
+    return (d && d->nq == 1 && d->tpc > 0 && d->tpc <= 3 && (d->ks[0] == 7 || d->ks[0] == 9) && (d->waves == 4 || d->waves == 8)) ? 1 : 0;
 }
 
 extern "C" int vg_conv_mm(const vg_mm_desc* d, const float* x, const float* a_img, const int32_t* tau, const int32_t* dlt,
@@ -455,6 +477,11 @@
     if (!x || !a_img || !tau || !dlt || !y) { vg_set_error("vg_conv_mm: null argument"); return VG_ERR_ARG; }
     if ((in_scale == nullptr) != (in_shift == nullptr) || (in_scale && d->per_group <= 0)) { vg_set_error("vg_conv_mm: in_scale/in_shift/per_group inconsistent"); return VG_ERR_ARG; }
     if (stats_part && (stats_per_group <= 0 || d->N % stats_per_group)) { vg_set_error("vg_conv_mm: bad statistics arguments"); return VG_ERR_ARG; }
+    const bool bns = d->bn_mean != nullptr || d->bn_rstd != nullptr;
+    if (bns) {
+        if (!d->bn_mean || !d->bn_rstd || !mask_src || !stats_part) { vg_set_error("vg_conv_mm: batch-norm sums need bn_mean, bn_rstd, mask_src and stats_part"); return VG_ERR_ARG; }
+        if (!vg_conv_mm_bnsums_ok(d)) { vg_set_error("vg_conv_mm: no batch-norm-sums instance for %d classes x %d k-steps", d->nq, d->ks[0]); return VG_ERR_UNSUPPORTED; }
+    }
     p.has_pro = (d->relu_in || in_scale) ? 1 : 0;
     hipStream_t s = (hipStream_t)stream;
     const int threads = d->waves * VG_WAVE;
@@ -468,14 +495,18 @@
     const bool db = d->dbuf != 0, mk = mask_src != nullptr, w4 = d->waves == 4;
 #define MM_LAUNCH_W(W, NQ, TPC, K0, K1, K2, K3) { \
         constexpr int OCC_ = (TPC * (K0 + K1 + K2 + K3) + 10 * TPC <= 96 && K0 > 0) ? 4 : 2; \
-        if (db) { if (mk) launch(conv_mm_k<W, NQ, TPC, K0, K1, K2, K3, true, OCC_, true>); else launch(conv_mm_k<W, NQ, TPC, K0, K1, K2, K3, true, OCC_, false>); } \
-        else    { if (mk) launch(conv_mm_k<W, NQ, TPC, K0, K1, K2, K3, false, OCC_, true>); else launch(conv_mm_k<W, NQ, TPC, K0, K1, K2, K3, false, OCC_, false>); } }
+        if (db) { if (mk) launch(conv_mm_k<W, NQ, TPC, K0, K1, K2, K3, true, OCC_, 1>); else launch(conv_mm_k<W, NQ, TPC, K0, K1, K2, K3, true, OCC_, 0>); } \
+        else    { if (mk) launch(conv_mm_k<W, NQ, TPC, K0, K1, K2, K3, false, OCC_, 1>); else launch(conv_mm_k<W, NQ, TPC, K0, K1, K2, K3, false, OCC_, 0>); } }
+#define MM_BNS_W(W, K0) { if (db) launch(conv_mm_k<W, 1, 3, K0, 0, 0, 0, true, 4, 2>); else launch(conv_mm_k<W, 1, 3, K0, 0, 0, 0, false, 4, 2>); }
+#define MM_BNS(K0) { if (w4) MM_BNS_W(4, K0) else MM_BNS_W(8, K0) }
 #define MM_LAUNCH(NQ, TPC, K0, K1, K2, K3) { if (w4) MM_LAUNCH_W(4, NQ, TPC, K0, K1, K2, K3) else MM_LAUNCH_W(8, NQ, TPC, K0, K1, K2, K3) }
 #define MM_TPC(NQ, K0, K1, K2, K3) \
     { if (d->tpc <= 3) MM_LAUNCH(NQ, 3, K0, K1, K2, K3) else if (d->tpc <= 4) MM_LAUNCH(NQ, 4, K0, K1, K2, K3) else if (d->tpc <= 5) MM_LAUNCH(NQ, 5, K0, K1, K2, K3) \
       else if (d->tpc <= 6) MM_LAUNCH(NQ, 6, K0, K1, K2, K3) else MM_LAUNCH(NQ, 8, K0, K1, K2, K3) }
     const int* k = d->ks;
-    if (d->nq == 1 && d->tpc <= 8) {
+    if (bns) {
+        if (k[0] == 7) MM_BNS(7) else MM_BNS(9)
+    } else if (d->nq == 1 && d->tpc <= 8) {
         if (k[0] == 7) MM_TPC(1, 7, 0, 0, 0)
         else if (k[0] == 9) MM_TPC(1, 9, 0, 0, 0)
         else if (k[0] == 12) MM_TPC(1, 12, 0, 0, 0)
@@ -487,6 +518,8 @@
         else if (k[0] == 2 && k[1] == 2 && k[2] == 2 && k[3] == 2) MM_LAUNCH(4, 4, 2, 2, 2, 2)
         else MM_LAUNCH(4, 4, 0, 0, 0, 0)
     } else { vg_set_error("vg_conv_mm: no kernel instance for %d classes x %d tiles per wave", d->nq, d->tpc); return VG_ERR_UNSUPPORTED; }
+#undef MM_BNS
+#undef MM_BNS_W
 #undef MM_TPC
 #undef MM_LAUNCH
 #undef MM_LAUNCH_W
diff --git a/vae-gam_amd/ops.py b/vae-gam_amd/ops.py
--- a/vae-gam_amd/ops.py
+++ b/vae-gam_amd/ops.py
@@ -41,6 +41,7 @@
 import os as _os
 SIDE_STREAM = bool(int(_os.environ.get('VG_SIDE_STREAM', '1')))
 FUSE_LAST_BN_BWD = bool(int(_os.environ.get('VG_FUSE_LAST_BN_BWD', '1')))
+DGRAD_BN_SUMS = bool(int(_os.environ.get('VG_DGRAD_BN_SUMS', '1')))
 WGRAD_BN_SUMS = bool(int(_os.environ.get('VG_WGRAD_BN_SUMS', '1')))
 FC_SIDE_STREAM = bool(int(_os.environ.get('VG_FC_SIDE_STREAM', '0')))
 _SIDE = {}
@@ -325,13 +326,25 @@
     return None
 
 
-def bn_backward_(dxe, p, gamma, mean, rstd, relu, per_group, sync=None, beta=None, producer_bias_grad=None):
+def bn_backward_(dxe, p, gamma, mean, rstd, relu, per_group, sync=None, beta=None, producer_bias_grad=None, pre=None):
     lib = _lib.get_lib()
     N, C = p.shape[0], p.shape[1]
     P = p[0, 0].numel()
     G = N // per_group
     ws = _bn_ws(p, N, C, P, per_group)
     sums = torch.empty((G * C, 2), dtype=torch.float64, device=p.device)
+    if producer_bias_grad is not None:
+        assert producer_bias_grad.shape == (C,) and producer_bias_grad.is_contiguous() and producer_bias_grad.dtype == torch.float32
+    if pre is not None:
+        assert sync is None, 'producer-side partials: single-GPU path'
+        assert pre.dtype == torch.float64 and pre.device == p.device and pre.numel() % (G * C * 2) == 0
+        gg, bg = _grad_buf(gamma), _grad_buf(beta)
+        acc = gg is not None and bg is not None
+        if not acc:
+            gg = torch.empty(C, dtype=torch.float32, device=p.device); bg = torch.empty_like(gg)
+        _call(p, 'vg_bn_bwd_apply_parts', _p(_chk(dxe)), _p(_chk(p)), N, C, P, per_group, int(relu), _p(gamma), _p(mean), _p(rstd), _p(pre),
+              pre.numel() // (G * C * 2), float(per_group * P), _p(sums), _p(ws), _p(producer_bias_grad), 1, _p(gg), _p(bg), int(acc))
+        return (None, None) if acc else (gg, bg)
     _call(p, 'vg_bn_bwd_reduce', _p(_chk(dxe)), _p(_chk(p)), N, C, P, per_group, int(relu), _p(mean), _p(rstd), _p(ws),
              _p(sums))
     count = float(per_group * P)
@@ -341,8 +354,6 @@
         sums = sync(sums)
         count = count * sync.world_size
     parts = torch.empty((2, G, C), dtype=torch.float32, device=p.device)
-    if producer_bias_grad is not None:
-        assert producer_bias_grad.shape == (C,) and producer_bias_grad.is_contiguous() and producer_bias_grad.dtype == torch.float32
     _call(p, 'vg_bn_bwd_apply', _p(dxe), _p(p), N, C, P, per_group, int(relu), _p(gamma), _p(mean), _p(rstd), _p(sums),
              count, _p(parts[0]), _p(parts[1]), _p(ws), _p(producer_bias_grad), 1)
     src = local if local is not None else sums
@@ -536,9 +547,13 @@
                 if dw_by_bn and wg is None:
                     dw = dw_t
             else:
-                dp = conv_mm(dy, mmb[0], mmb[1], None, False, None, None, 1, None) if mmb is not None else \
-                    conv_backward_data(dy, wb, spec, in_size, None)
-                dgamma, dbeta = bn_backward_(dp, p_in, gamma, mean, rstd, relu_in, per_group, ctx.sync, beta, pbg)
+                pre = None
+                if DGRAD_BN_SUMS and mmb is not None and ctx.sync is None and mmb[0].bn_sums_ok():
+                    dp, pre = conv_mm(dy, mmb[0], mmb[1], None, False, None, None, 1, None, bn_sums=(p_in, mean, rstd, relu_in, per_group))
+                else:
+                    dp = conv_mm(dy, mmb[0], mmb[1], None, False, None, None, 1, None) if mmb is not None else \
+                        conv_backward_data(dy, wb, spec, in_size, None)
+                dgamma, dbeta = bn_backward_(dp, p_in, gamma, mean, rstd, relu_in, per_group, ctx.sync, beta, pbg, pre=pre)
         else:
             msk = p_in if relu_in else None
             dp = conv_mm(dy, mmb[0], mmb[1], None, False, None, None, 1, msk) if mmb is not None else \
@@ -1041,6 +1056,11 @@
             d.oh0[q] = int(self.oh0[q]) if q < self.nq else 0
             d.ow0[q] = int(self.ow0[q]) if q < self.nq else 0
         return d
+
+    def bn_sums_ok(self):
+        if '_bns' not in self.__dict__:
+            self._bns = bool(_lib.get_lib().dll.vg_conv_mm_bnsums_ok(ctypes.byref(self.desc(1, False, 1))))
+        return self._bns
 
     def gather(self, weight):
         _, _, aidx = self.tables(weight.device)
@@ -1223,7 +1243,7 @@
                   tau=tau.reshape(-1), dlt=dlt.reshape(-1), aidx=aidx, mode=mode)
 
 
-def conv_mm(x, plan: MmPlan, aimg, bias, relu_in, scale, shift, per_group, mask_src=None, next_bn=None):
+def conv_mm(x, plan: MmPlan, aimg, bias, relu_in, scale, shift, per_group, mask_src=None, next_bn=None, bn_sums=None):
     lib = _lib.get_lib()
     N = x.shape[0]
     assert tuple(x.shape[1:]) == (plan.CI, plan.ID, plan.IH, plan.IW), (tuple(x.shape), plan.CI, plan.ID, plan.IH, plan.IW)
@@ -1231,6 +1251,17 @@
     d = plan.desc(N, relu_in, per_group if scale is not None else 1)
     y = torch.empty((N, plan.CO, plan.OD, plan.OH, plan.OW), dtype=torch.float32, device=x.device)
     _chk(x); _chk(aimg)
+    if bn_sums is not None:
+        p, mean, rstd, bn_relu, bn_pg = bn_sums
+        assert mask_src is None and not next_bn and tuple(p.shape) == tuple(y.shape) and N % int(bn_pg) == 0
+        G = N // int(bn_pg)
+        assert mean.numel() == G * plan.CO and rstd.numel() == G * plan.CO
+        d.bn_mean, d.bn_rstd = _chk(mean).data_ptr(), _chk(rstd).data_ptr()
+        chunks = lib.size('vg_conv_mm_stats_chunks', ctypes.byref(d), int(bn_pg))
+        part = torch.empty(G * plan.CO * chunks * 2, dtype=torch.float64, device=x.device)
+        _call(x, 'vg_conv_mm', ctypes.byref(d), _p(x), _p(aimg), _p(tau), _p(dlt), _p(bias), _p(scale), _p(shift), _p(_chk(p)), _p(y),
+              int(bn_pg), int(bool(bn_relu)), _p(part))
+        return y, part
     if next_bn:
         chunks = lib.size('vg_conv_mm_stats_chunks', ctypes.byref(d), int(next_bn))
         G = N // int(next_bn)
```

Result: no change. 10000 volumes/s (-0.2%).
